# mhamilton723/STEGO

Hardware: NVIDIA H100
Metric: train-step images/sec (higher is better)
Workload: dtype bf16

## Files before the change

include/stego_b200.h:

```cpp
#ifndef STEGO_B200_H_
#define STEGO_B200_H_

#ifdef __cplusplus
extern "C" {
#endif

#define STEGO_API

STEGO_API int stego_version(void);
STEGO_API const char* stego_last_error(void);
STEGO_API long long stego_launch_count(void);

STEGO_API int stego_gemm_bf16(const void* A, int lda, int a_mn_major, const void* B, int ldb, int b_mn_major,
                              int M, int N, int K, void* out, int ldo, int out_bf16, const float* bias, int act,
                              const float* residual, int ldr, int row_div, int splits, int atomic_out,
                              void* stream);

STEGO_API int stego_gemm_bf16_batched(const void* A, int lda, long long a_batch_stride, int a_mn_major, const void* B,
                                      int ldb, long long b_batch_stride, int b_mn_major, int batch, int M, int N, int K,
                                      void* out, int ldo, long long out_batch_stride, int out_bf16, const float* bias,
                                      int act, void* stream);

STEGO_API int stego_vit_patchify(const float* img, void* out_bf16, int B, int H, int W, int patch, void* stream);
STEGO_API int stego_vit_patchify_bf16(const void* img_bf16, void* out_bf16, int B, int H, int W, int patch,
                                      void* stream);
STEGO_API int stego_vit_patchify_tta(const void* img, int img_is_bf16, void* out_bf16, int B, int H, int W, int patch,
                                     void* stream);
STEGO_API int stego_vit_cls_rows(float* x, const float* cls_token, const float* pos_embed, int B, int ntok, int E,
                                 void* stream);
STEGO_API int stego_layernorm_bf16(const float* x, const float* gamma, const float* beta, void* out_bf16, int rows,
                                   int E, float eps, int drop_cls_ntok, void* stream);
STEGO_API int stego_layernorm_gap(const float* x, const float* gamma, const float* beta, float* out, int B, int ntok,
                                  int E, float eps, void* stream);
STEGO_API int stego_linear_rows_f32(const float* x, const void* w_bf16, int ldw, const float* bias, float* out, int B,
                                    int N, int K, void* stream);
STEGO_API int stego_attention_fwd(const void* qkv, void* out, int B, int N, int E, int heads, void* stream);
STEGO_API int stego_attention_probs(const void* qkv, float* probs, int B, int N, int E, int heads, void* stream);

STEGO_API int stego_sample_norm_fwd(const void* src, const void* src_pos, int src_is_bf16, long long stride_b,
                                    long long stride_c, long long stride_y, long long stride_x,
                                    const float* chan_scale, const float* chan_scale_pos, const float* coords1,
                                    const float* coords2, const long long* perms, void* tiles, int B, int C,
                                    int Cpad, int H, int W, int feature_samples, int nslots, int perms_are_raw_randperm,
                                    void* stream);
STEGO_API int stego_sample_labels_fwd(const void* label, const void* label_pos, int label_bytes, const float* coords1,
                                      const float* coords2, const long long* perms, void* tiles, int B, int n_classes,
                                      int Cpad, int H, int W, int feature_samples, int nslots,
                                      int perms_are_raw_randperm, void* stream);
STEGO_API int stego_corr_loss_fwd(const void* feat_tiles, const void* code_tiles, int B, int feature_samples, int E,
                                  int D, int nslots, int ncalls, const int* slot_of_call_host,
                                  const float* shifts_host, int pointwise, int zero_clamp, int stabilize,
                                  float* partials, float* stats, float* cd_out, float* fdc_out, float* loss_out,
                                  void* stream);
STEGO_API int stego_corr_loss_bwd(const void* feat_tiles, const void* code_tiles, int B, int feature_samples, int E,
                                  int D, int nslots, int ncalls, const int* slot_of_call_host,
                                  const float* shifts_host, int pointwise, int zero_clamp, int stabilize,
                                  const float* stats, const float* gscale, const float* gelem, const float* gcd,
                                  float* dtiles, void* stream);
STEGO_API int stego_sample_norm_bwd(const float* code, const float* code_pos, long long stride_b, long long stride_c,
                                    long long stride_y, long long stride_x, const float* coords1,
                                    const float* coords2, const long long* perms, const float* dtiles, float* dcode,
                                    float* dcode_pos, int B, int C, int H, int W, int feature_samples, int nslots,
                                    int perms_are_raw_randperm, void* stream);

STEGO_API int stego_corr_loss_tiled_fwd(const void* feat_tiles, const void* code_tiles, int B, int feature_samples,
                                        int E, int D, int nslots, int ncalls, const int* slot_of_call_host,
                                        const float* shifts_host, int pointwise, int zero_clamp, int stabilize,
                                        float* row_partials, float* row_means, float* stats, float* cd_out,
                                        float* fdc_out, float* loss_out, void* stream);
STEGO_API int stego_corr_loss_tiled_bwd(const void* feat_tiles, const void* code_tiles, int B, int feature_samples,
                                        int E, int D, int nslots, int ncalls, const int* slot_of_call_host,
                                        const float* shifts_host, int pointwise, int zero_clamp, int stabilize,
                                        const float* stats, const float* row_means, const float* gscale,
                                        const float* gelem, const float* gcd, float* dtiles, void* stream);

STEGO_API int stego_salience_counts(const void* salience, const void* salience_pos, int mask_bytes, int B, int H, int W,
                                    int* counts, void* stream);
STEGO_API int stego_salience_coords(const void* salience, const void* salience_pos, int mask_bytes, int B, int H, int W,
                                    int feature_samples, long long seed, const long long* offsets,
                                    const void* draws_u32, const float* u_reg1, const float* u_reg2,
                                    const float* u_keep, float* coords1, float* coords2, void* scratch, void* stream);
STEGO_API long long stego_salience_scratch_bytes(int B, int H, int W);

STEGO_API int stego_aug_record_words(void);
STEGO_API long long stego_aug_scratch_bytes(int B, int size);
STEGO_API int stego_aug_views(const float* img, long long stride_b, long long stride_c, long long stride_y,
                              long long stride_x, int B, int H, int W, int size, const int* records, void* scratch,
                              float* img_aug, float* coord_aug, void* stream);

STEGO_API int stego_frames_rgb8(const void* staging_host, const void* staging_dev, long long bytes,
                                long long table_words, int B, int res, float mean0, float mean1, float mean2,
                                float std0, float std1, float std2, float* out, void* stream);
STEGO_API int stego_labels_u8(const void* staging_host, const void* staging_dev, long long bytes,
                              long long table_words, int B, int res, const long long* lut, long long* out, void* stream);
STEGO_API int stego_frames_store_rgb8(const void* staging_host, const void* staging_dev, long long bytes,
                                      long long table_words, int B, int res, unsigned char* store, long long n,
                                      long long r0, void* stream);
STEGO_API int stego_labels_store_u8(const void* staging_host, const void* staging_dev, long long bytes,
                                    long long table_words, int B, int res, unsigned char* store, long long n,
                                    long long r0, void* stream);
STEGO_API int stego_dataset_batch(const unsigned char* images, const unsigned char* labels, long long n, int res,
                                  const long long* index, int count, const long long* lut, float mean0, float mean1,
                                  float mean2, float std0, float std1, float std2, int out_bf16, int mask_kind,
                                  void* img, long long* label, void* mask, void* stream);
STEGO_API int stego_evalset_batch(const unsigned char* images, const unsigned char* labels, long long n, int res,
                                  const long long* index, int count, const long long* lut, float mean0, float mean1,
                                  float mean2, float std0, float std1, float std2, int out_bf16, int mask_kind,
                                  void* img, long long* label, void* mask, void* stream);
STEGO_API int stego_store_rows_u8(const void* staging_host, const void* staging_dev, long long bytes,
                                  long long table_words, int B, int channels, unsigned char* store,
                                  long long store_bytes, void* stream);
STEGO_API int stego_store_batch_window(const unsigned char* images, long long image_bytes,
                                       const unsigned char* labels, long long label_bytes, const long long* rows,
                                       long long n, int res, const long long* record, int count,
                                       const long long* lut, float mean0, float mean1, float mean2, float std0,
                                       float std1, float std2, int out_bf16, int mask_kind, void* img,
                                       long long* label, void* mask, void* stream);

STEGO_API int stego_jpeg_crops_codec(const void* staging_host, const void* staging_dev, long long bytes,
                                     long long table_words, int count, unsigned char* workspace,
                                     long long workspace_bytes, void* stream);
STEGO_API int stego_jpeg_crops_store_rgb8(const void* staging_host, const void* staging_dev, long long bytes,
                                          long long table_words, int count, int res, const unsigned char* workspace,
                                          long long workspace_bytes, unsigned char* store, long long n, long long r0,
                                          void* stream);

STEGO_API int stego_tb_tables(double* edges, float* thresholds);
STEGO_API int stego_tb_histogram(const float* values, long long n, const float* thresholds, long long* counts,
                                 double* cta_partials, double* stats, void* stream);
STEGO_API int stego_corr_loss_fwd_hist(const void* feat_tiles, const void* code_tiles, int B, int feature_samples,
                                       int E, int D, int nslots, int ncalls, const int* slot_of_call_host,
                                       const float* shifts_host, int pointwise, int zero_clamp, int stabilize,
                                       float* partials, float* stats, float* cd_out, float* fdc_out, float* loss_out,
                                       const float* thresholds, long long* hist_counts, double* hist_cta_partials,
                                       double* hist_stats, void* stream);
STEGO_API int stego_corr_loss_tiled_fwd_hist(const void* feat_tiles, const void* code_tiles, int B,
                                             int feature_samples, int E, int D, int nslots, int ncalls,
                                             const int* slot_of_call_host, const float* shifts_host, int pointwise,
                                             int zero_clamp, int stabilize, float* row_partials, float* row_means,
                                             float* stats, float* cd_out, float* fdc_out, float* loss_out,
                                             const float* thresholds, long long* hist_counts,
                                             double* hist_cta_partials, double* hist_stats, void* stream);

#define STEGO_PR_BINS 4096
STEGO_API int stego_sample_label_ids(const void* label, int label_bytes, const float* coords1, const float* coords2,
                                     int* ids, int B, int n_classes, int H, int W, int feature_samples, void* stream);
STEGO_API int stego_corr_pr(const void* feat_tiles, const void* code_tiles, const int* ids, long long* counts, int B,
                            int feature_samples, int E, int D, void* stream);

STEGO_API int stego_heatmap_prep_target(const void* target, int target_is_bf16, long long stride_b, long long stride_c,
                                        long long stride_y, long long stride_x, int B, int E, int h, int w, int Epad,
                                        void* ops, float* inv_norm, void* stream);
STEGO_API int stego_heatmap_sample_queries(const void* feats, int feats_is_bf16, long long stride_b, long long stride_c,
                                           long long stride_y, long long stride_x, const float* points, int B, int P,
                                           int E, int h, int w, int Epad, int nseg, void* ops, void* stream);
STEGO_API int stego_heatmap_finish(float* corr, const float* inv_norm, int B, int P, int hw, void* stream);
STEGO_API int stego_heatmap_upsample(const float* in, float* out, long long n, int h, int w, int H, int W, void* stream);

STEGO_API int stego_head_dropout3(const void* feat_bf16, const float* mask1, const float* mask2, const float* mask3,
                                  void* out1, void* out2, void* out3, int B, int hw, int E, void* stream);
STEGO_API int stego_cast_pad_bf16(const float* in, int ld_in, int C, void* out_bf16, int ld_out, long long rows,
                                  void* stream);
STEGO_API int stego_relu_bwd_bf16(const float* dh, const void* h_bf16, void* out_bf16, long long n, void* stream);
STEGO_API int stego_colsum(const void* in, int in_is_bf16, int ld, int C, long long rows, float* out, void* stream);
STEGO_API int stego_adam_step(float* param, const float* grad, float* exp_avg, float* exp_avg_sq, long long n,
                              double lr, double beta1, double beta2, double eps, int step, float grad_scale,
                              void* stream);

STEGO_API int stego_step_losses(const float* corr_stats, int ncalls, const float* call_weights_host,
                                const float* extra0, const float* extra1, float* out4, void* stream);

STEGO_API int stego_cluster_lookup_fwd(const float* x, long long stride_b, long long stride_c, long long stride_pix,
                                       const float* clusters, int B, int C, int n_classes, long long npix,
                                       int use_alpha, float alpha, long long* assign, float* probs, float* log_probs,
                                       float* loss_out, float* scratch, void* stream);
STEGO_API int stego_cluster_lookup_bwd(const float* x, long long stride_b, long long stride_c, long long stride_pix,
                                       const float* clusters, int B, int C, int n_classes, long long npix,
                                       int use_alpha, float alpha, const float* grad_loss_dev,
                                       float* dnc_scratch, float* dclusters, void* stream);
STEGO_API int stego_linear_probe_ce(const float* code, long long ld_code, int C, const float* W, const float* bias,
                                    int n_classes, const void* label, int label_bytes, int B, int h, int w, int H,
                                    int Wimg, float* logits_scratch, float* dlogits_scratch, float* partials_scratch,
                                    float* loss_out, float grad_loss, float* dW, float* db, void* stream);
STEGO_API int stego_linear_probe_ce_wide(const float* code, long long ld_code, int C, const float* W, const float* bias,
                                         int n_classes, const void* label, int label_bytes, int B, int h, int w, int H,
                                         int Wimg, float* logits_scratch, float* dlogits_scratch,
                                         long long* dfix_scratch, float* partials_scratch, float* loss_out,
                                         float grad_loss, float* dW, float* db, void* stream);
STEGO_API int stego_cluster_lookup_wide(const float* x, long long ld_x, long long rows, int C, const float* clusters,
                                        int n_classes, int* assign_scratch, float* inv_scratch, float* partials_scratch,
                                        float* loss_out, float* dnc_scratch, float* dclusters, void* stream);

STEGO_API int stego_eval_probes(const float* code, const float* code_flip, long long ld_code, int C, int B, int h, int w,
                                int H, int W, const float* lin_weight, const float* lin_bias, int n_lin,
                                const float* clusters, int n_clu, float alpha, float* lr_scratch, float* lin_log_probs,
                                float* clu_log_probs, unsigned char* lin_argmax, unsigned char* clu_argmax,
                                const void* label, int label_bytes, int n_label_classes, long long* lin_confusion,
                                long long* clu_confusion, void* stream);
STEGO_API int stego_eval_probes_mosaic(const float* code, const float* code_flip, long long ld_code, int C, int B, int h,
                                       int w, int H, int W, const float* lin_weight, const float* lin_bias, int n_lin,
                                       const float* clusters, int n_clu, float alpha, float* lr_scratch,
                                       float* lin_log_probs, float* clu_log_probs, unsigned char* lin_argmax,
                                       unsigned char* clu_argmax, const void* label, int label_bytes,
                                       int n_label_classes, long long* lin_confusion, long long* clu_confusion,
                                       int tile0, int tile_rows, int tiles_per_row, long long pitch, void* stream);

STEGO_API int stego_knn_topk(const float* feats, int n, int E, int k, void* planes_scratch, long long* idx_out,
                             float* val_out, void* stream);
STEGO_API int stego_knn_prep(const float* feats, int n, int E, void* planes, void* stream);
STEGO_API int stego_knn_topk_rows(const void* planes, int n, int E, int k, int row0, int nrows, long long* idx_out,
                                  float* val_out, void* stream);

STEGO_API int stego_crf_lattice(int H, int W, int d, float sxy, float srgb, const unsigned char* image, long long* keys,
                                float* bary, void* stream);
STEGO_API int stego_crf_unary(const float* logits, float* unary, float* Q, long long N, int C, void* stream);
STEGO_API int stego_crf_norm(int d, long long N, int M, const int* offset, const float* bary, const int* rowptr,
                             const int* slots, const int* n1, const int* n2, float* values, float* values_tmp,
                             float* norm_out, void* stream);
STEGO_API int stego_crf_mean_field(int B, long long N, int n_lin, int n_clu, int n_iter, const float* unary, float* Q,
                                   const int* off_g, const float* bary_g, const int* rowptr_g, const int* slots_g,
                                   const int* n1_g, const int* n2_g, const float* norm_g, int Mg,
                                   const int* off_b, const float* bary_b, const int* rowptr_b, const int* slots_b,
                                   const int* n1_b, const int* n2_b, const float* norm_b, int Mb, float w_g,
                                   float w_b, float* val_g, float* tmp_g, float* val_b, float* tmp_b, float* lin_q,
                                   float* clu_q, unsigned char* lin_pred, unsigned char* clu_pred,
                                   const void* label, int label_bytes, int n_label_classes, long long* lin_conf,
                                   long long* clu_conf, void* stream);

STEGO_API int stego_eval_crf_unary(const float* code, const float* code_flip, long long ld_code, int C, int B, int h, int w,
                                   int H, int W, const float* lin_weight, const float* lin_bias, int n_lin,
                                   const float* clusters, int n_clu, float alpha, float* lr_scratch, float* unary, float* Q,
                                   void* stream);
STEGO_API int stego_eval_crf_unary_mosaic(const float* code, const float* code_flip, long long ld_code, int C, int B,
                                          int h, int w, int H, int W, const float* lin_weight, const float* lin_bias,
                                          int n_lin, const float* clusters, int n_clu, float alpha, float* lr_scratch,
                                          float* unary, float* Q, int probes, int tile0, int tile_rows,
                                          int tiles_per_row, long long pitch, void* stream);

STEGO_API int stego_eval_probes_bf16(const void* code, const void* code_flip, long long ld_code, int C, int B, int h,
                                     int w, int H, int W, const float* lin_weight, const float* lin_bias, int n_lin,
                                     const float* clusters, int n_clu, float alpha, float* lr_scratch,
                                     float* lin_log_probs, float* clu_log_probs, unsigned char* lin_argmax,
                                     unsigned char* clu_argmax, const void* label, int label_bytes,
                                     int n_label_classes, long long* lin_confusion, long long* clu_confusion,
                                     void* stream);
STEGO_API int stego_eval_probes_mosaic_bf16(const void* code, const void* code_flip, long long ld_code, int C, int B,
                                            int h, int w, int H, int W, const float* lin_weight, const float* lin_bias,
                                            int n_lin, const float* clusters, int n_clu, float alpha,
                                            float* lr_scratch, float* lin_log_probs, float* clu_log_probs,
                                            unsigned char* lin_argmax, unsigned char* clu_argmax, const void* label,
                                            int label_bytes, int n_label_classes, long long* lin_confusion,
                                            long long* clu_confusion, int tile0, int tile_rows, int tiles_per_row,
                                            long long pitch, void* stream);
STEGO_API int stego_eval_crf_unary_bf16(const void* code, const void* code_flip, long long ld_code, int C, int B, int h,
                                        int w, int H, int W, const float* lin_weight, const float* lin_bias, int n_lin,
                                        const float* clusters, int n_clu, float alpha, float* lr_scratch, float* unary,
                                        float* Q, void* stream);
STEGO_API int stego_eval_crf_unary_mosaic_bf16(const void* code, const void* code_flip, long long ld_code, int C, int B,
                                               int h, int w, int H, int W, const float* lin_weight,
                                               const float* lin_bias, int n_lin, const float* clusters, int n_clu,
                                               float alpha, float* lr_scratch, float* unary, float* Q, int probes,
                                               int tile0, int tile_rows, int tiles_per_row, long long pitch,
                                               void* stream);

STEGO_API int stego_crf_loss_fwd(const float* guidance, long long g_sb, long long g_sc, long long g_sy, long long g_sx, int Cg,
                                 const float* clusters, long long c_sb, long long c_sc, long long c_sy, long long c_sx, int C,
                                 const long long* coords, int B, int n, int H, int W, float alpha, float beta, float gamma,
                                 float w1, float w2, float shift, float* sel, float* gsel, int* pos, float* out, void* stream);
STEGO_API int stego_crf_loss_bwd(const float* grad_out, const float* sel, const float* gsel, const int* pos,
                                 const long long* coords, int B, int C, int n, float alpha, float beta, float gamma, float w1,
                                 float w2, float shift, float* dsel, float* dclusters, long long c_sb, long long c_sc,
                                 long long c_sy, long long c_sx, void* stream);

STEGO_API int stego_cosine_fwd(const float* a, long long a_sb, long long a_sc, long long a_sy, long long a_sx, const float* b,
                               long long b_sb, long long b_sc, long long b_sy, long long b_sx, int B, int C, int H, int W,
                               float eps, float* cosv, float* norma, float* normb, void* stream);
STEGO_API int stego_cosine_bwd(const float* a, long long a_sb, long long a_sc, long long a_sy, long long a_sx, const float* b,
                               long long b_sb, long long b_sc, long long b_sy, long long b_sx, int B, int C, int H, int W,
                               float eps, const float* cosv, const float* norma, const float* normb, const float* grad_cos,
                               float* da, float* db, void* stream);

STEGO_API int stego_aug_align_fwd(const float* coord_aug, int S, const float* code, long long sb, long long sc,
                                  long long sy, long long sx, int B, int C, int h, float* grid, float* sampled,
                                  void* stream);
STEGO_API int stego_aug_align_bwd(const float* grid, const float* dsampled, int B, int C, int h, float* dcode,
                                  long long sb, long long sc, long long sy, long long sx, void* stream);
STEGO_API int stego_aug_align_loss(const float* cosv, long long n, float weight, float* loss, float* total, void* stream);

STEGO_API int stego_rec_fwd(const float* code, long long ldc, const void* feat, long long ldf, const float* m3, int hw,
                            const float* weight, const float* bias, long long M, int E, int D, float* cosv, float* nr,
                            float* nf, void* stream);
STEGO_API long long stego_rec_scratch_bytes(long long M, int E, int D);
STEGO_API int stego_rec_bwd(const float* code, long long ldc, const void* feat, long long ldf, const float* m3, int hw,
                            const float* weight, const float* bias, long long M, int E, int D, const float* cosv,
                            const float* nr, const float* nf, const float* dcos, float* dcode, long long ldd,
                            float* scratch, long long scratch_bytes, float* dweight, float* dbias, void* stream);

STEGO_API int stego_crf_guidance(const float* img, long long sb, long long sc, long long sy, long long sx, int Cg, int H,
                                 int W, const long long* coords, int B, int n, int S, float* gsel, int* pos, void* stream);
STEGO_API int stego_crf_mean_fwd(const float* code, long long sb, long long sc, long long sy, long long sx, int C, int h,
                                 int w, const long long* coords, int B, int n, int S, float alpha, float beta, float gamma,
                                 float w1, float w2, float shift, const float* gsel, const int* pos, float* raw,
                                 float* sel, float* nrm, double* tile_sum, void* stream);
STEGO_API int stego_crf_mean_loss(const double* tile_sum, int B, int n, float weight, float* loss, float* total,
                                  void* stream);
STEGO_API int stego_crf_mean_bwd(const float* gscalar, const float* sel, const float* nrm, const float* gsel,
                                 const int* pos, const long long* coords, int B, int C, int n, int h, int w, int S,
                                 float alpha, float beta, float gamma, float w1, float w2, float shift, float* dsel,
                                 float* dcode, long long sb, long long sc, long long sy, long long sx, void* stream);

STEGO_API int stego_p2p_alloc(long long bytes, long long* ptr_out, unsigned char* handle_out);
STEGO_API int stego_p2p_open(const unsigned char* handle, long long* ptr_out);
STEGO_API int stego_p2p_close(long long ptr);
STEGO_API int stego_p2p_free(long long ptr);
STEGO_API int stego_p2p_publish(const float* grad, long long n, float* export_slot, const long long* peer_flags, int rank,
                                int world, int epoch, int* status, int timeout_ms, void* stream);
STEGO_API int stego_p2p_adam(const long long* peer_exports, int world, float* param, float* grad, float* exp_avg,
                             float* exp_avg_sq, long long n, const double* group_desc, int ngroups, float grad_scale,
                             void* stream);

#ifdef __cplusplus
}
#endif
#endif
```

stego_b200/_lib.py:

```python
from __future__ import annotations

import ctypes
import gc
import os
import re
import threading
from typing import Dict, List, Tuple

import torch

_HERE = os.path.dirname(os.path.abspath(__file__))
LIB_PATH = os.path.join(_HERE, "libstego_b200.so")
HEADER_PATH = os.path.join(_HERE, "..", "include", "stego_b200.h")

_lib = None
replayed_launches = 0

_CTYPES = {
    "int": ctypes.c_int,
    "float": ctypes.c_float,
    "double": ctypes.c_double,
    "long long": ctypes.c_longlong,
    "void*": ctypes.c_void_p,
    "const void*": ctypes.c_void_p,
    "const float*": ctypes.c_void_p,
    "float*": ctypes.c_void_p,
    "const long long*": ctypes.c_void_p,
    "long long*": ctypes.c_void_p,
    "const int*": ctypes.c_void_p,
    "int*": ctypes.c_void_p,
    "const char*": ctypes.c_char_p,
    "unsigned char*": ctypes.c_void_p,
    "const unsigned char*": ctypes.c_void_p,
    "const double*": ctypes.c_void_p,
    "double*": ctypes.c_void_p,
}


def header_prototypes() -> Dict[str, Tuple[str, List[str]]]:
    text = open(HEADER_PATH).read()
    text = re.sub(r"/\*.*?\*/", "", text, flags=re.S)
    text = re.sub(r"//[^\n]*", "", text)
    text = re.sub(r"^\s*#[^\n]*", "", text, flags=re.M)
    protos: Dict[str, Tuple[str, List[str]]] = {}
    for m in re.finditer(r"STEGO_API\s+([\w\s\*]+?)\s*\b(stego_\w+)\s*\(([^;]*?)\)\s*;", text, flags=re.S):
        ret, name, args = m.group(1).strip(), m.group(2), m.group(3).strip()
        arg_types: List[str] = []
        if args and args != "void":
            for a in args.split(","):
                a = " ".join(a.split())
                t = re.sub(r"\s*\b\w+$", "", a).strip()
                t = t.replace(" *", "*")
                arg_types.append(t)
        protos[name] = (ret.replace(" *", "*"), arg_types)
    return protos


def load():
    global _lib
    if _lib is not None:
        return _lib
    if not os.path.exists(LIB_PATH):
        raise RuntimeError(
            f"stego_b200: {LIB_PATH} is missing. Build it with `python -m stego_b200.build` "
            "(or __graft_entry__.build()). There is no CPU / eager fallback for the hot path.")
    lib = ctypes.CDLL(LIB_PATH)
    for name, (ret, args) in header_prototypes().items():
        fn = getattr(lib, name)
        fn.restype = _CTYPES[ret]
        fn.argtypes = [_CTYPES[a] for a in args]
    _lib = lib
    return lib


def launch_count() -> int:
    return int(load().stego_launch_count()) + replayed_launches


_CAPTURE_LOCK = threading.Lock()


_CAPTURE_STREAMS: Dict[int, torch.cuda.Stream] = {}


def capture_stream(device: torch.device) -> torch.cuda.Stream:
    if device.index not in _CAPTURE_STREAMS:
        _CAPTURE_STREAMS[device.index] = torch.cuda.Stream(device=device)
    return _CAPTURE_STREAMS[device.index]


class Graph:

    def __init__(self, fn):
        self.device = torch.device("cuda", torch.cuda.current_device())
        with _CAPTURE_LOCK, torch.cuda.device(self.device):
            self._capture(fn)

    def _capture(self, fn):
        torch.cuda.synchronize()
        gc.collect()
        enabled = gc.isenabled()
        gc.disable()
        try:
            self.graph = torch.cuda.CUDAGraph()
            n0 = load().stego_launch_count()
            with torch.cuda.graph(self.graph, stream=capture_stream(self.device)):
                self.result = fn()
            self.launches = load().stego_launch_count() - n0
        finally:
            if enabled:
                gc.enable()

    def replay(self) -> None:
        global replayed_launches
        if torch.cuda.current_device() == self.device.index:
            self.graph.replay()
        else:
            with torch.cuda.device(self.device):
                self.graph.replay()
        replayed_launches += self.launches


def last_error() -> str:
    return load().stego_last_error().decode("utf-8", "replace")


def check(rc: int, what: str) -> None:
    if rc != 0:
        raise RuntimeError(f"stego_b200.{what} failed with status {rc}: {last_error()}")


def ptr(t) -> int:
    if t is None:
        return 0
    return t.data_ptr()


def stream() -> int:
    return torch.cuda.current_stream().cuda_stream


def require_cuda(*tensors) -> None:
    for t in tensors:
        if t is not None and not t.is_cuda:
            raise RuntimeError("stego_b200: hot-path tensors must live on a CUDA device (no CPU fallback)")
```

stego_b200/csrc/attention.cu:

```cuda
#include <stdlib.h>

#include "common.cuh"
#include "host_util.h"

namespace stego {

constexpr int ATT_BQ = 128;
constexpr int ATT_BKV = 64;
constexpr int ATT_D = 64;
constexpr int ATT_STAGES = 4;
constexpr int ATT_THREADS = 288;

constexpr uint32_t ATT_Q_BYTES = 128 * 64 * 2;
constexpr uint32_t ATT_KV_BYTES = 64 * 64 * 2;
constexpr uint32_t ATT_SMEM_Q = 0;
constexpr uint32_t ATT_SMEM_KV = ATT_Q_BYTES;
constexpr uint32_t ATT_SMEM_BAR = ATT_SMEM_KV + ATT_STAGES * 2 * ATT_KV_BYTES;
constexpr uint32_t ATT_SMEM_TOTAL = ATT_SMEM_BAR + 128;

struct AttnParams {
  int N;
  int E;
  float scale_log2e;
};

__global__ void __launch_bounds__(ATT_THREADS, 2)
attention_fwd_kernel(const __grid_constant__ CUtensorMap tmQKV, const __grid_constant__ CUtensorMap tmOut, AttnParams p) {
  extern __shared__ __align__(1024) uint8_t smem[];
  if ((smem_u32(smem) & 1023u) != 0u) __trap();
  uint64_t* bars = reinterpret_cast<uint64_t*>(smem + ATT_SMEM_BAR);
  uint64_t* q_full = bars;
  uint64_t* kv_full = bars + 1;
  uint64_t* kv_empty = kv_full + ATT_STAGES;

  const int warp = threadIdx.x >> 5;
  const int lane = threadIdx.x & 31;
  const int q0 = blockIdx.x * ATT_BQ;
  const int head = blockIdx.y;
  const int img = blockIdx.z;
  const int nkv = (p.N + ATT_BKV - 1) / ATT_BKV;

  if (threadIdx.x == 0) {
    mbar_init(q_full, 1);
    for (int s = 0; s < ATT_STAGES; ++s) {
      mbar_init(&kv_full[s], 1);
      mbar_init(&kv_empty[s], 2);
    }
    fence_barrier_init();
  }
  __syncthreads();

  if (warp == 8) {
    if (lane == 0) {
      tma_prefetch_desc(&tmQKV);
      tma_prefetch_desc(&tmOut);
      mbar_arrive_expect_tx(q_full, ATT_Q_BYTES);
      tma_load_3d(smem + ATT_SMEM_Q, &tmQKV, q_full, head * ATT_D, q0, img);
      tma_load_3d(smem + ATT_SMEM_Q + ATT_Q_BYTES / 2, &tmQKV, q_full, head * ATT_D, q0 + 64, img);
      uint32_t stage = 0, phase = 0;
      for (int j = 0; j < nkv; ++j) {
        mbar_wait(&kv_empty[stage], phase ^ 1u);
        uint8_t* sk = smem + ATT_SMEM_KV + stage * 2 * ATT_KV_BYTES;
        mbar_arrive_expect_tx(&kv_full[stage], 2 * ATT_KV_BYTES);
        tma_load_3d(sk, &tmQKV, &kv_full[stage], p.E + head * ATT_D, j * ATT_BKV, img);
        tma_load_3d(sk + ATT_KV_BYTES, &tmQKV, &kv_full[stage], 2 * p.E + head * ATT_D, j * ATT_BKV, img);
        if (++stage == ATT_STAGES) { stage = 0; phase ^= 1u; }
      }
    }
    return;
  }

  const int wg = warp >> 2;
  const int wq = warp & 3;
  const bool leader = (threadIdx.x & 127) == 0;
  const float c = p.scale_log2e;
  constexpr uint32_t DESC_HI = smem_desc_hi_sw128(1024);
  uint8_t* sq = smem + ATT_SMEM_Q + wg * (ATT_Q_BYTES / 2);
  const uint32_t q_lo = smem_desc_lo(smem_u32(sq), 16);
  const uint32_t k_lo0 = smem_desc_lo(smem_u32(smem + ATT_SMEM_KV), 16);
  const uint32_t v_lo0 = smem_desc_lo(smem_u32(smem + ATT_SMEM_KV + ATT_KV_BYTES), 8192);
  float o[32];
#pragma unroll
  for (int i = 0; i < 32; ++i) o[i] = 0.f;
  float m_run[2] = {-INFINITY, -INFINITY}, l_run[2] = {0.f, 0.f};
  mbar_wait(q_full, 0);
  uint32_t stage = 0, phase = 0;
  for (int j = 0; j < nkv; ++j) {
    mbar_wait(&kv_full[stage], phase);
    const uint32_t k_lo = k_lo0 + stage * ((2 * ATT_KV_BYTES) >> 4);
    const uint32_t v_lo = v_lo0 + stage * ((2 * ATT_KV_BYTES) >> 4);
    float s[32];
    wgmma_fence();
#pragma unroll
    for (uint32_t k = 0; k < ATT_D / 16; ++k)
      wgmma_ss<64, 0, 0>(s, smem_desc_join(q_lo + k * 2, DESC_HI), smem_desc_join(k_lo + k * 2, DESC_HI), k > 0 ? 1u : 0u);
    wgmma_commit();
    wgmma_wait<0>();
    fence_operands(s);
    const int valid = p.N - j * ATT_BKV;
    if (valid < ATT_BKV) {
#pragma unroll
      for (int i = 0; i < 32; ++i)
        if (8 * (i >> 2) + 2 * (lane & 3) + (i & 1) >= valid) s[i] = -INFINITY;
    }
    float alpha[2], mc[2];
#pragma unroll
    for (int h = 0; h < 2; ++h) {
      float mx = -INFINITY;
#pragma unroll
      for (int i = 0; i < 8; ++i) mx = fmaxf(mx, fmaxf(s[4 * i + 2 * h], s[4 * i + 2 * h + 1]));
      mx = fmaxf(mx, __shfl_xor_sync(0xffffffffu, mx, 1));
      mx = fmaxf(mx, __shfl_xor_sync(0xffffffffu, mx, 2));
      const float m_new = fmaxf(m_run[h], mx);
      alpha[h] = ex2_approx((m_run[h] - m_new) * c);
      m_run[h] = m_new;
      mc[h] = m_new * c;
    }
    uint32_t a[4][4];
    float rs[2] = {0.f, 0.f};
#pragma unroll
    for (int i = 0; i < 8; ++i) {
#pragma unroll
      for (int h = 0; h < 2; ++h) {
        const float e0 = ex2_approx(fmaf(s[4 * i + 2 * h], c, -mc[h]));
        const float e1 = ex2_approx(fmaf(s[4 * i + 2 * h + 1], c, -mc[h]));
        rs[h] += e0 + e1;
        a[i >> 1][(i & 1) * 2 + h] = pack_bf16x2(e0, e1);
      }
    }
#pragma unroll
    for (int h = 0; h < 2; ++h) l_run[h] = l_run[h] * alpha[h] + rs[h];
#pragma unroll
    for (int i = 0; i < 32; ++i) o[i] *= alpha[(i >> 1) & 1];
    wgmma_fence();
#pragma unroll
    for (uint32_t kk = 0; kk < ATT_BKV / 16; ++kk)
      wgmma_rs_n64<1>(o, a[kk], smem_desc_join(v_lo + kk * (2048u >> 4), DESC_HI), 1u);
    wgmma_commit();
    wgmma_wait<0>();
    fence_operands(o);
    if (leader) mbar_arrive(&kv_empty[stage]);
    if (++stage == ATT_STAGES) { stage = 0; phase ^= 1u; }
  }
  float inv[2];
#pragma unroll
  for (int h = 0; h < 2; ++h) {
    float l = l_run[h];
    l += __shfl_xor_sync(0xffffffffu, l, 1);
    l += __shfl_xor_sync(0xffffffffu, l, 2);
    inv[h] = __fdividef(1.0f, l);
  }
#pragma unroll
  for (int i = 0; i < 8; ++i) {
#pragma unroll
    for (int h = 0; h < 2; ++h) {
      const uint32_t r = static_cast<uint32_t>(wq * 16 + (lane >> 2) + 8 * h);
      const uint32_t off = sw128_offset(r, static_cast<uint32_t>(i)) + 4u * static_cast<uint32_t>(lane & 3);
      *reinterpret_cast<uint32_t*>(sq + off) = pack_bf16x2(o[4 * i + 2 * h] * inv[h], o[4 * i + 2 * h + 1] * inv[h]);
    }
  }
  fence_proxy_async_smem();
  asm volatile("bar.sync %0, 128;\n" ::"r"(wg + 1) : "memory");
  if (leader) {
    tma_store_3d(sq, &tmOut, head * ATT_D, q0 + wg * 64, img);
    tma_commit_group();
    tma_wait_group_read<0>();
  }
}

constexpr int PRB_STAGES = 4;
constexpr int PRB_PITCH = 72;
constexpr uint32_t PRB_SMEM_K = ATT_Q_BYTES;
constexpr uint32_t PRB_SMEM_STAGE = PRB_SMEM_K + PRB_STAGES * ATT_KV_BYTES;
constexpr uint32_t PRB_WARP_STAGE_BYTES = 16 * PRB_PITCH * 4;
constexpr uint32_t PRB_SMEM_BAR = PRB_SMEM_STAGE + 8 * PRB_WARP_STAGE_BYTES;
constexpr uint32_t PRB_SMEM_TOTAL = PRB_SMEM_BAR + 128;

__device__ __forceinline__ void st_global_cs(float* p, float v) {
  asm volatile("st.global.cs.f32 [%0], %1;\n" ::"l"(p), "f"(v) : "memory");
}

__global__ void __launch_bounds__(ATT_THREADS, 2)
attention_probs_kernel(const __grid_constant__ CUtensorMap tmQKV, float* __restrict__ probs, AttnParams p) {
  extern __shared__ __align__(1024) uint8_t smem[];
  if ((smem_u32(smem) & 1023u) != 0u) __trap();
  uint64_t* bars = reinterpret_cast<uint64_t*>(smem + PRB_SMEM_BAR);
  uint64_t* q_full = bars;
  uint64_t* k_full = bars + 1;
  uint64_t* k_empty = k_full + PRB_STAGES;

  const int warp = threadIdx.x >> 5;
  const int lane = threadIdx.x & 31;
  const int q0 = blockIdx.x * ATT_BQ;
  const int head = blockIdx.y;
  const int img = blockIdx.z;
  const int nkv = (p.N + ATT_BKV - 1) / ATT_BKV;

  if (threadIdx.x == 0) {
    mbar_init(q_full, 1);
    for (int s = 0; s < PRB_STAGES; ++s) {
      mbar_init(&k_full[s], 1);
      mbar_init(&k_empty[s], 2);
    }
    fence_barrier_init();
  }
  __syncthreads();

  if (warp == 8) {
    if (lane == 0) {
      tma_prefetch_desc(&tmQKV);
      mbar_arrive_expect_tx(q_full, ATT_Q_BYTES);
      tma_load_3d(smem, &tmQKV, q_full, head * ATT_D, q0, img);
      tma_load_3d(smem + ATT_Q_BYTES / 2, &tmQKV, q_full, head * ATT_D, q0 + 64, img);
      uint32_t stage = 0, phase = 0;
      for (int j = 0; j < 2 * nkv; ++j) {
        mbar_wait(&k_empty[stage], phase ^ 1u);
        mbar_arrive_expect_tx(&k_full[stage], ATT_KV_BYTES);
        tma_load_3d(smem + PRB_SMEM_K + stage * ATT_KV_BYTES, &tmQKV, &k_full[stage], p.E + head * ATT_D,
                    (j < nkv ? j : j - nkv) * ATT_BKV, img);
        if (++stage == PRB_STAGES) { stage = 0; phase ^= 1u; }
      }
    }
    return;
  }

  const int wg = warp >> 2;
  const int wq = warp & 3;
  const bool leader = (threadIdx.x & 127) == 0;
  const float c = p.scale_log2e;
  constexpr uint32_t DESC_HI = smem_desc_hi_sw128(1024);
  const uint32_t q_lo = smem_desc_lo(smem_u32(smem + wg * (ATT_Q_BYTES / 2)), 16);
  const uint32_t k_lo0 = smem_desc_lo(smem_u32(smem + PRB_SMEM_K), 16);
  float* stage_tile = reinterpret_cast<float*>(smem + PRB_SMEM_STAGE + warp * PRB_WARP_STAGE_BYTES);
  const int row0 = q0 + wg * 64 + wq * 16;
  float m_run[2] = {-INFINITY, -INFINITY}, l_run[2] = {0.f, 0.f};
  float inv[2] = {0.f, 0.f};
  mbar_wait(q_full, 0);
  uint32_t stage = 0, phase = 0;
  for (int j = 0; j < 2 * nkv; ++j) {
    const bool store_pass = j >= nkv;
    const int kt = store_pass ? j - nkv : j;
    mbar_wait(&k_full[stage], phase);
    const uint32_t k_lo = k_lo0 + stage * (ATT_KV_BYTES >> 4);
    float s[32];
    wgmma_fence();
#pragma unroll
    for (uint32_t k = 0; k < ATT_D / 16; ++k)
      wgmma_ss<64, 0, 0>(s, smem_desc_join(q_lo + k * 2, DESC_HI), smem_desc_join(k_lo + k * 2, DESC_HI), k > 0 ? 1u : 0u);
    wgmma_commit();
    wgmma_wait<0>();
    fence_operands(s);
    if (leader) mbar_arrive(&k_empty[stage]);
    if (++stage == PRB_STAGES) { stage = 0; phase ^= 1u; }
    const int valid = p.N - kt * ATT_BKV;
    if (!store_pass) {
      if (valid < ATT_BKV) {
#pragma unroll
        for (int i = 0; i < 32; ++i)
          if (8 * (i >> 2) + 2 * (lane & 3) + (i & 1) >= valid) s[i] = -INFINITY;
      }
#pragma unroll
      for (int h = 0; h < 2; ++h) {
        float mx = -INFINITY;
#pragma unroll
        for (int i = 0; i < 8; ++i) mx = fmaxf(mx, fmaxf(s[4 * i + 2 * h], s[4 * i + 2 * h + 1]));
        mx = fmaxf(mx, __shfl_xor_sync(0xffffffffu, mx, 1));
        mx = fmaxf(mx, __shfl_xor_sync(0xffffffffu, mx, 2));
        const float m_new = fmaxf(m_run[h], mx);
        const float alpha = ex2_approx((m_run[h] - m_new) * c);
        float rs = 0.f;
#pragma unroll
        for (int i = 0; i < 8; ++i)
          rs += ex2_approx((s[4 * i + 2 * h] - m_new) * c) + ex2_approx((s[4 * i + 2 * h + 1] - m_new) * c);
        l_run[h] = l_run[h] * alpha + rs;
        m_run[h] = m_new;
      }
      if (kt == nkv - 1) {
#pragma unroll
        for (int h = 0; h < 2; ++h) {
          float l = l_run[h];
          l += __shfl_xor_sync(0xffffffffu, l, 1);
          l += __shfl_xor_sync(0xffffffffu, l, 2);
          inv[h] = __frcp_rn(l);
        }
      }
      continue;
    }
    __syncwarp();
#pragma unroll
    for (int i = 0; i < 8; ++i) {
#pragma unroll
      for (int h = 0; h < 2; ++h) {
        const float p0 = ex2_approx((s[4 * i + 2 * h] - m_run[h]) * c) * inv[h];
        const float p1 = ex2_approx((s[4 * i + 2 * h + 1] - m_run[h]) * c) * inv[h];
        float2* dst = reinterpret_cast<float2*>(stage_tile + ((lane >> 2) + 8 * h) * PRB_PITCH + 8 * i + 2 * (lane & 3));
        *dst = make_float2(p0, p1);
      }
    }
    __syncwarp();
    const int nrows = min(16, p.N - row0);
    const size_t plane = (static_cast<size_t>(img) * gridDim.y + head) * static_cast<size_t>(p.N);
    float* out = probs + (plane + static_cast<size_t>(row0)) * static_cast<size_t>(p.N) + static_cast<size_t>(kt) * ATT_BKV;
#pragma unroll 4
    for (int r = 0; r < nrows; ++r) {
      float* orow = out + static_cast<size_t>(r) * static_cast<size_t>(p.N);
      if (lane < valid) st_global_cs(orow + lane, stage_tile[r * PRB_PITCH + lane]);
      if (lane + 32 < valid) st_global_cs(orow + lane + 32, stage_tile[r * PRB_PITCH + lane + 32]);
    }
  }
}

}

using namespace stego;

extern "C" int stego_attention_fwd(const void* qkv, void* out, int B, int N, int E, int heads, void* stream_) {
  cudaStream_t stream = reinterpret_cast<cudaStream_t>(stream_);
  STEGO_CHECK_ARG(qkv && out, "stego_attention_fwd: null pointer");
  STEGO_CHECK_ARG(B > 0 && N > 0 && heads > 0, "stego_attention_fwd: bad sizes");
  STEGO_CHECK_ARG(E == heads * ATT_D, "stego_attention_fwd: head_dim must be 64 (E=%d heads=%d)", E, heads);
  STEGO_CHECK_ARG((reinterpret_cast<uintptr_t>(out) & 15u) == 0, "stego_attention_fwd: out not 16-byte aligned");
  CUtensorMap tm;
  uint64_t dims[3] = {(uint64_t)3 * E, (uint64_t)N, (uint64_t)B};
  uint64_t str[2] = {(uint64_t)3 * E * 2, (uint64_t)N * 3 * E * 2};
  uint32_t box[3] = {64, 64, 1};
  int rc = make_tmap_bf16(&tm, qkv, 3, dims, str, box);
  if (rc != STEGO_OK) return rc;
  CUtensorMap tmo;
  uint64_t odims[3] = {(uint64_t)E, (uint64_t)N, (uint64_t)B};
  uint64_t ostr[2] = {(uint64_t)E * 2, (uint64_t)N * E * 2};
  if ((rc = make_tmap_bf16(&tmo, out, 3, odims, ostr, box)) != STEGO_OK) return rc;
  if ((rc = opt_in_smem<attention_fwd_kernel>(ATT_SMEM_TOTAL, "attention_fwd_kernel")) != STEGO_OK) return rc;
  AttnParams p;
  p.N = N;
  p.E = E;
  p.scale_log2e = 0.125f * 1.4426950408889634f;
  dim3 grid((N + ATT_BQ - 1) / ATT_BQ, heads, B);
  attention_fwd_kernel<<<grid, ATT_THREADS, ATT_SMEM_TOTAL, stream>>>(tm, tmo, p);
  STEGO_CHECK_LAUNCH("attention_fwd_kernel");
  return STEGO_OK;
}

extern "C" int stego_attention_probs(const void* qkv, float* probs, int B, int N, int E, int heads, void* stream_) {
  cudaStream_t stream = reinterpret_cast<cudaStream_t>(stream_);
  STEGO_CHECK_ARG(qkv && probs, "stego_attention_probs: null pointer");
  STEGO_CHECK_ARG(B > 0 && N > 0 && heads > 0, "stego_attention_probs: bad sizes");
  STEGO_CHECK_ARG(B <= 65535 && heads <= 65535, "stego_attention_probs: B and heads must be <= 65535");
  STEGO_CHECK_ARG(E == heads * ATT_D, "stego_attention_probs: head_dim must be 64 (E=%d heads=%d)", E, heads);
  STEGO_CHECK_ARG((reinterpret_cast<uintptr_t>(probs) & 3u) == 0, "stego_attention_probs: probs not 4-byte aligned");
  CUtensorMap tm;
  uint64_t dims[3] = {(uint64_t)3 * E, (uint64_t)N, (uint64_t)B};
  uint64_t str[2] = {(uint64_t)3 * E * 2, (uint64_t)N * 3 * E * 2};
  uint32_t box[3] = {64, 64, 1};
  int rc = make_tmap_bf16(&tm, qkv, 3, dims, str, box);
  if (rc != STEGO_OK) return rc;
  if ((rc = opt_in_smem<attention_probs_kernel>(PRB_SMEM_TOTAL, "attention_probs_kernel")) != STEGO_OK) return rc;
  AttnParams p;
  p.N = N;
  p.E = E;
  p.scale_log2e = 0.125f * 1.4426950408889634f;
  dim3 grid((N + ATT_BQ - 1) / ATT_BQ, heads, B);
  attention_probs_kernel<<<grid, ATT_THREADS, PRB_SMEM_TOTAL, stream>>>(tm, probs, p);
  STEGO_CHECK_LAUNCH("attention_probs_kernel");
  return STEGO_OK;
}
```

stego_b200/csrc/common.cuh:

```cuda
#pragma once
#include <cuda.h>
#include <cuda_bf16.h>
#include <cuda_runtime.h>
#include <stdint.h>
#include <stdio.h>

namespace stego {

typedef __nv_bfloat16 bf16;

__device__ __forceinline__ uint32_t smem_u32(const void* p) {
  return static_cast<uint32_t>(__cvta_generic_to_shared(p));
}
__device__ __forceinline__ uint32_t lane_id() { return threadIdx.x & 31u; }

__device__ __forceinline__ float warp_sum(float v) {
#pragma unroll
  for (int o = 16; o > 0; o >>= 1) v += __shfl_xor_sync(0xffffffffu, v, o);
  return v;
}
__device__ __forceinline__ float warp_max(float v) {
#pragma unroll
  for (int o = 16; o > 0; o >>= 1) v = fmaxf(v, __shfl_xor_sync(0xffffffffu, v, o));
  return v;
}

__device__ __forceinline__ void mbar_init(uint64_t* bar, uint32_t count) {
  asm volatile("mbarrier.init.shared::cta.b64 [%0], %1;\n" ::"r"(smem_u32(bar)), "r"(count) : "memory");
}
__device__ __forceinline__ void fence_barrier_init() {
  asm volatile("fence.mbarrier_init.release.cluster;\n" ::: "memory");
}
__device__ __forceinline__ void fence_proxy_async_smem() {
  asm volatile("fence.proxy.async.shared::cta;\n" ::: "memory");
}
__device__ __forceinline__ void mbar_arrive(uint64_t* bar) {
  asm volatile("mbarrier.arrive.shared::cta.b64 _, [%0];\n" ::"r"(smem_u32(bar)) : "memory");
}
__device__ __forceinline__ void mbar_arrive_expect_tx(uint64_t* bar, uint32_t bytes) {
  asm volatile("mbarrier.arrive.expect_tx.shared::cta.b64 _, [%0], %1;\n" ::"r"(smem_u32(bar)), "r"(bytes)
               : "memory");
}
__device__ __forceinline__ bool mbar_try_wait(uint64_t* bar, uint32_t parity) {
  uint32_t ok;
  asm volatile(
      "{\n\t.reg .pred P1;\n\t"
      "mbarrier.try_wait.parity.shared::cta.b64 P1, [%1], %2, %3;\n\t"
      "selp.b32 %0, 1, 0, P1;\n\t}\n"
      : "=r"(ok)
      : "r"(smem_u32(bar)), "r"(parity), "r"(1000000u)
      : "memory");
  return ok != 0;
}

__device__ __forceinline__ bool mbar_test_wait(uint64_t* bar, uint32_t parity) {
  uint32_t ok;
  asm volatile(
      "{\n\t.reg .pred P1;\n\t"
      "mbarrier.test_wait.parity.shared::cta.b64 P1, [%1], %2;\n\t"
      "selp.b32 %0, 1, 0, P1;\n\t}\n"
      : "=r"(ok)
      : "r"(smem_u32(bar)), "r"(parity)
      : "memory");
  return ok != 0;
}

#ifndef STEGO_MBAR_TIMEOUT_NS
#define STEGO_MBAR_TIMEOUT_NS 4000000000ull
#endif
__device__ __forceinline__ uint64_t globaltimer_ns() {
  uint64_t t;
  asm volatile("mov.u64 %0, %%globaltimer;\n" : "=l"(t));
  return t;
}
__device__ __forceinline__ void mbar_wait(uint64_t* bar, uint32_t parity) {
  if (mbar_test_wait(bar, parity)) return;
  if (mbar_try_wait(bar, parity)) return;
  uint32_t spins = 0;
  uint64_t t0 = 0;
  while (!mbar_try_wait(bar, parity)) {
    if ((++spins & 0x3Fu) == 0) {
      const uint64_t now = globaltimer_ns();
      if (t0 == 0) {
        t0 = now;
      } else if (now - t0 > STEGO_MBAR_TIMEOUT_NS) {
        __trap();
      }
    }
  }
}

__device__ __forceinline__ void tma_prefetch_desc(const CUtensorMap* m) {
  asm volatile("prefetch.tensormap [%0];\n" ::"l"(reinterpret_cast<uint64_t>(m)) : "memory");
}
__device__ __forceinline__ void tma_load_2d(void* smem_dst, const CUtensorMap* m, uint64_t* bar, int c0, int c1) {
  asm volatile(
      "cp.async.bulk.tensor.2d.shared::cluster.global.mbarrier::complete_tx::bytes [%0], [%1, {%3, %4}], [%2];\n" ::"r"(
          smem_u32(smem_dst)),
      "l"(reinterpret_cast<uint64_t>(m)), "r"(smem_u32(bar)), "r"(c0), "r"(c1)
      : "memory");
}
__device__ __forceinline__ void tma_load_3d(void* smem_dst, const CUtensorMap* m, uint64_t* bar, int c0, int c1,
                                            int c2) {
  asm volatile(
      "cp.async.bulk.tensor.3d.shared::cluster.global.mbarrier::complete_tx::bytes [%0], [%1, {%3, %4, %5}], "
      "[%2];\n" ::"r"(smem_u32(smem_dst)),
      "l"(reinterpret_cast<uint64_t>(m)), "r"(smem_u32(bar)), "r"(c0), "r"(c1), "r"(c2)
      : "memory");
}

__device__ __forceinline__ void tma_prefetch_l2_2d(const CUtensorMap* m, int c0, int c1) {
  asm volatile("cp.async.bulk.prefetch.tensor.2d.L2.global [%0, {%1, %2}];\n" ::"l"(reinterpret_cast<uint64_t>(m)),
               "r"(c0), "r"(c1)
               : "memory");
}

__device__ __forceinline__ void tma_store_3d(uint32_t smem_src, const CUtensorMap* m, int c0, int c1, int c2) {
  asm volatile("cp.async.bulk.tensor.3d.global.shared::cta.bulk_group [%0, {%2, %3, %4}], [%1];\n" ::"l"(
                   reinterpret_cast<uint64_t>(m)),
               "r"(smem_src), "r"(c0), "r"(c1), "r"(c2)
               : "memory");
}
__device__ __forceinline__ void tma_store_3d(const void* smem_src, const CUtensorMap* m, int c0, int c1, int c2) {
  tma_store_3d(smem_u32(smem_src), m, c0, c1, c2);
}
__device__ __forceinline__ void tma_reduce_add_3d(uint32_t smem_src, const CUtensorMap* m, int c0, int c1, int c2) {
  asm volatile("cp.reduce.async.bulk.tensor.3d.global.shared::cta.add.bulk_group [%0, {%2, %3, %4}], [%1];\n" ::"l"(
                   reinterpret_cast<uint64_t>(m)),
               "r"(smem_src), "r"(c0), "r"(c1), "r"(c2)
               : "memory");
}

__device__ __forceinline__ void st_shared_b32(uint32_t addr, uint32_t v) {
  asm volatile("st.shared.b32 [%0], %1;\n" ::"r"(addr), "r"(v) : "memory");
}
__device__ __forceinline__ void st_shared_v2_f32(uint32_t addr, float a, float b) {
  asm volatile("st.shared.v2.f32 [%0], {%1, %2};\n" ::"r"(addr), "f"(a), "f"(b) : "memory");
}
__device__ __forceinline__ void tma_commit_group() { asm volatile("cp.async.bulk.commit_group;\n" ::: "memory"); }
template <int kPending>
__device__ __forceinline__ void tma_wait_group_read() {
  asm volatile("cp.async.bulk.wait_group.read %0;\n" ::"n"(kPending) : "memory");
}
template <int kPending>
__device__ __forceinline__ void tma_wait_group() {
  asm volatile("cp.async.bulk.wait_group %0;\n" ::"n"(kPending) : "memory");
}

__device__ __forceinline__ void named_bar_sync(int id, int threads) {
  asm volatile("bar.sync %0, %1;\n" ::"r"(id), "r"(threads) : "memory");
}

__device__ __forceinline__ void wgmma_fence() { asm volatile("wgmma.fence.sync.aligned;\n" ::: "memory"); }
__device__ __forceinline__ void wgmma_commit() { asm volatile("wgmma.commit_group.sync.aligned;\n" ::: "memory"); }
template <int kPending>
__device__ __forceinline__ void wgmma_wait() {
  asm volatile("wgmma.wait_group.sync.aligned %0;\n" ::"n"(kPending) : "memory");
}
template <int kN>
__device__ __forceinline__ void fence_operands(float (&d)[kN]) {
#pragma unroll
  for (int i = 0; i < kN; ++i) asm volatile("" : "+f"(d[i])::"memory");
}

template <int kTransA, int kTransB>
__device__ __forceinline__ void wgmma_ss_n64(float (&d)[32], uint64_t desc_a, uint64_t desc_b, uint32_t accumulate) {
  asm volatile(
      "{\n\t.reg .pred p;\n\tsetp.ne.b32 p, %34, 0;\n\t"
      "wgmma.mma_async.sync.aligned.m64n64k16.f32.bf16.bf16 {%0, %1, %2, %3, %4, %5, %6, %7, %8, %9, %10, %11, %12, %13, %14, %15, %16, %17, %18, %19, %20, %21, %22, %23, %24, %25, %26, %27, %28, %29, %30, %31}, %32, %33, p, 1, 1, %35, %36;\n\t}\n"
      : "+f"(d[0]), "+f"(d[1]), "+f"(d[2]), "+f"(d[3]), "+f"(d[4]), "+f"(d[5]), "+f"(d[6]), "+f"(d[7]), "+f"(d[8]), "+f"(d[9]), "+f"(d[10]), "+f"(d[11]), "+f"(d[12]), "+f"(d[13]), "+f"(d[14]), "+f"(d[15]), "+f"(d[16]), "+f"(d[17]), "+f"(d[18]), "+f"(d[19]), "+f"(d[20]), "+f"(d[21]), "+f"(d[22]), "+f"(d[23]), "+f"(d[24]), "+f"(d[25]), "+f"(d[26]), "+f"(d[27]), "+f"(d[28]), "+f"(d[29]), "+f"(d[30]), "+f"(d[31])
      : "l"(desc_a), "l"(desc_b), "r"(accumulate), "n"(kTransA), "n"(kTransB));
}

template <int kTransA, int kTransB>
__device__ __forceinline__ void wgmma_ss_n128(float (&d)[64], uint64_t desc_a, uint64_t desc_b, uint32_t accumulate) {
  asm volatile(
      "{\n\t.reg .pred p;\n\tsetp.ne.b32 p, %66, 0;\n\t"
      "wgmma.mma_async.sync.aligned.m64n128k16.f32.bf16.bf16 {%0, %1, %2, %3, %4, %5, %6, %7, %8, %9, %10, %11, %12, %13, %14, %15, %16, %17, %18, %19, %20, %21, %22, %23, %24, %25, %26, %27, %28, %29, %30, %31, %32, %33, %34, %35, %36, %37, %38, %39, %40, %41, %42, %43, %44, %45, %46, %47, %48, %49, %50, %51, %52, %53, %54, %55, %56, %57, %58, %59, %60, %61, %62, %63}, %64, %65, p, 1, 1, %67, %68;\n\t}\n"
      : "+f"(d[0]), "+f"(d[1]), "+f"(d[2]), "+f"(d[3]), "+f"(d[4]), "+f"(d[5]), "+f"(d[6]), "+f"(d[7]), "+f"(d[8]), "+f"(d[9]), "+f"(d[10]), "+f"(d[11]), "+f"(d[12]), "+f"(d[13]), "+f"(d[14]), "+f"(d[15]), "+f"(d[16]), "+f"(d[17]), "+f"(d[18]), "+f"(d[19]), "+f"(d[20]), "+f"(d[21]), "+f"(d[22]), "+f"(d[23]), "+f"(d[24]), "+f"(d[25]), "+f"(d[26]), "+f"(d[27]), "+f"(d[28]), "+f"(d[29]), "+f"(d[30]), "+f"(d[31]), "+f"(d[32]), "+f"(d[33]), "+f"(d[34]), "+f"(d[35]), "+f"(d[36]), "+f"(d[37]), "+f"(d[38]), "+f"(d[39]), "+f"(d[40]), "+f"(d[41]), "+f"(d[42]), "+f"(d[43]), "+f"(d[44]), "+f"(d[45]), "+f"(d[46]), "+f"(d[47]), "+f"(d[48]), "+f"(d[49]), "+f"(d[50]), "+f"(d[51]), "+f"(d[52]), "+f"(d[53]), "+f"(d[54]), "+f"(d[55]), "+f"(d[56]), "+f"(d[57]), "+f"(d[58]), "+f"(d[59]), "+f"(d[60]), "+f"(d[61]), "+f"(d[62]), "+f"(d[63])
      : "l"(desc_a), "l"(desc_b), "r"(accumulate), "n"(kTransA), "n"(kTransB));
}

template <int kTransA, int kTransB>
__device__ __forceinline__ void wgmma_ss_n256(float (&d)[128], uint64_t desc_a, uint64_t desc_b, uint32_t accumulate) {
  asm volatile(
      "{\n\t.reg .pred p;\n\tsetp.ne.b32 p, %130, 0;\n\t"
      "wgmma.mma_async.sync.aligned.m64n256k16.f32.bf16.bf16 {%0, %1, %2, %3, %4, %5, %6, %7, %8, %9, %10, %11, %12, %13, %14, %15, %16, %17, %18, %19, %20, %21, %22, %23, %24, %25, %26, %27, %28, %29, %30, %31, %32, %33, %34, %35, %36, %37, %38, %39, %40, %41, %42, %43, %44, %45, %46, %47, %48, %49, %50, %51, %52, %53, %54, %55, %56, %57, %58, %59, %60, %61, %62, %63, %64, %65, %66, %67, %68, %69, %70, %71, %72, %73, %74, %75, %76, %77, %78, %79, %80, %81, %82, %83, %84, %85, %86, %87, %88, %89, %90, %91, %92, %93, %94, %95, %96, %97, %98, %99, %100, %101, %102, %103, %104, %105, %106, %107, %108, %109, %110, %111, %112, %113, %114, %115, %116, %117, %118, %119, %120, %121, %122, %123, %124, %125, %126, %127}, %128, %129, p, 1, 1, %131, %132;\n\t}\n"
      : "+f"(d[0]), "+f"(d[1]), "+f"(d[2]), "+f"(d[3]), "+f"(d[4]), "+f"(d[5]), "+f"(d[6]), "+f"(d[7]), "+f"(d[8]), "+f"(d[9]), "+f"(d[10]), "+f"(d[11]), "+f"(d[12]), "+f"(d[13]), "+f"(d[14]), "+f"(d[15]), "+f"(d[16]), "+f"(d[17]), "+f"(d[18]), "+f"(d[19]), "+f"(d[20]), "+f"(d[21]), "+f"(d[22]), "+f"(d[23]), "+f"(d[24]), "+f"(d[25]), "+f"(d[26]), "+f"(d[27]), "+f"(d[28]), "+f"(d[29]), "+f"(d[30]), "+f"(d[31]), "+f"(d[32]), "+f"(d[33]), "+f"(d[34]), "+f"(d[35]), "+f"(d[36]), "+f"(d[37]), "+f"(d[38]), "+f"(d[39]), "+f"(d[40]), "+f"(d[41]), "+f"(d[42]), "+f"(d[43]), "+f"(d[44]), "+f"(d[45]), "+f"(d[46]), "+f"(d[47]), "+f"(d[48]), "+f"(d[49]), "+f"(d[50]), "+f"(d[51]), "+f"(d[52]), "+f"(d[53]), "+f"(d[54]), "+f"(d[55]), "+f"(d[56]), "+f"(d[57]), "+f"(d[58]), "+f"(d[59]), "+f"(d[60]), "+f"(d[61]), "+f"(d[62]), "+f"(d[63]), "+f"(d[64]), "+f"(d[65]), "+f"(d[66]), "+f"(d[67]), "+f"(d[68]), "+f"(d[69]), "+f"(d[70]), "+f"(d[71]), "+f"(d[72]), "+f"(d[73]), "+f"(d[74]), "+f"(d[75]), "+f"(d[76]), "+f"(d[77]), "+f"(d[78]), "+f"(d[79]), "+f"(d[80]), "+f"(d[81]), "+f"(d[82]), "+f"(d[83]), "+f"(d[84]), "+f"(d[85]), "+f"(d[86]), "+f"(d[87]), "+f"(d[88]), "+f"(d[89]), "+f"(d[90]), "+f"(d[91]), "+f"(d[92]), "+f"(d[93]), "+f"(d[94]), "+f"(d[95]), "+f"(d[96]), "+f"(d[97]), "+f"(d[98]), "+f"(d[99]), "+f"(d[100]), "+f"(d[101]), "+f"(d[102]), "+f"(d[103]), "+f"(d[104]), "+f"(d[105]), "+f"(d[106]), "+f"(d[107]), "+f"(d[108]), "+f"(d[109]), "+f"(d[110]), "+f"(d[111]), "+f"(d[112]), "+f"(d[113]), "+f"(d[114]), "+f"(d[115]), "+f"(d[116]), "+f"(d[117]), "+f"(d[118]), "+f"(d[119]), "+f"(d[120]), "+f"(d[121]), "+f"(d[122]), "+f"(d[123]), "+f"(d[124]), "+f"(d[125]), "+f"(d[126]), "+f"(d[127])
      : "l"(desc_a), "l"(desc_b), "r"(accumulate), "n"(kTransA), "n"(kTransB));
}

template <int kTransB>
__device__ __forceinline__ void wgmma_rs_n64(float (&d)[32], const uint32_t (&a)[4], uint64_t desc_b, uint32_t accumulate) {
  asm volatile(
      "{\n\t.reg .pred p;\n\tsetp.ne.b32 p, %37, 0;\n\t"
      "wgmma.mma_async.sync.aligned.m64n64k16.f32.bf16.bf16 {%0, %1, %2, %3, %4, %5, %6, %7, %8, %9, %10, %11, %12, %13, %14, %15, %16, %17, %18, %19, %20, %21, %22, %23, %24, %25, %26, %27, %28, %29, %30, %31}, {%32, %33, %34, %35}, %36, p, 1, 1, %38;\n\t}\n"
      : "+f"(d[0]), "+f"(d[1]), "+f"(d[2]), "+f"(d[3]), "+f"(d[4]), "+f"(d[5]), "+f"(d[6]), "+f"(d[7]), "+f"(d[8]), "+f"(d[9]), "+f"(d[10]), "+f"(d[11]), "+f"(d[12]), "+f"(d[13]), "+f"(d[14]), "+f"(d[15]), "+f"(d[16]), "+f"(d[17]), "+f"(d[18]), "+f"(d[19]), "+f"(d[20]), "+f"(d[21]), "+f"(d[22]), "+f"(d[23]), "+f"(d[24]), "+f"(d[25]), "+f"(d[26]), "+f"(d[27]), "+f"(d[28]), "+f"(d[29]), "+f"(d[30]), "+f"(d[31])
      : "r"(a[0]), "r"(a[1]), "r"(a[2]), "r"(a[3]), "l"(desc_b), "r"(accumulate), "n"(kTransB));
}

template <int N, int kTransA, int kTransB>
__device__ __forceinline__ void wgmma_ss(float (&d)[N / 2], uint64_t desc_a, uint64_t desc_b, uint32_t accumulate) {
  static_assert(N == 64 || N == 128 || N == 256, "wgmma_ss: N must be 64, 128 or 256");
  if constexpr (N == 64) wgmma_ss_n64<kTransA, kTransB>(d, desc_a, desc_b, accumulate);
  else if constexpr (N == 128) wgmma_ss_n128<kTransA, kTransB>(d, desc_a, desc_b, accumulate);
  else wgmma_ss_n256<kTransA, kTransB>(d, desc_a, desc_b, accumulate);
}

template <uint32_t kRegs>
__device__ __forceinline__ void warpgroup_reg_alloc() { asm volatile("setmaxnreg.inc.sync.aligned.u32 %0;\n" ::"n"(kRegs)); }
template <uint32_t kRegs>
__device__ __forceinline__ void warpgroup_reg_dealloc() { asm volatile("setmaxnreg.dec.sync.aligned.u32 %0;\n" ::"n"(kRegs)); }

__device__ __forceinline__ float ex2_approx(float x) {
  float y;
  asm("ex2.approx.ftz.f32 %0, %1;\n" : "=f"(y) : "f"(x));
  return y;
}

__device__ __forceinline__ float ex2_approx_v(float x) {
  float y;
  asm volatile("ex2.approx.ftz.f32 %0, %1;\n" : "=f"(y) : "f"(x));
  return y;
}

__device__ __forceinline__ uint32_t smem_desc_lo(uint32_t smem_addr, uint32_t lbo_bytes) {
  return ((smem_addr & 0x3FFFFu) >> 4) | (((lbo_bytes >> 4) & 0x3FFFu) << 16);
}
__host__ __device__ constexpr uint32_t smem_desc_hi_sw128(uint32_t sbo_bytes) {
  return ((sbo_bytes >> 4) & 0x3FFFu) | (1u << 30);
}
__device__ __forceinline__ uint64_t smem_desc_join(uint32_t lo, uint32_t hi) {
  return (static_cast<uint64_t>(hi) << 32) | lo;
}

__device__ __forceinline__ uint32_t sw128_offset(uint32_t row, uint32_t chunk16) {
  return row * 128u + ((chunk16 ^ (row & 7u)) << 4);
}

__device__ __forceinline__ uint64_t pack_f32x2(float lo, float hi) {
  uint64_t r;
  asm("mov.b64 %0, {%1, %2};\n" : "=l"(r) : "f"(lo), "f"(hi));
  return r;
}
__device__ __forceinline__ void unpack_f32x2(uint64_t v, float& lo, float& hi) {
  asm("mov.b64 {%0, %1}, %2;\n" : "=f"(lo), "=f"(hi) : "l"(v));
}
__device__ __forceinline__ uint64_t fma_f32x2(uint64_t a, uint64_t b, uint64_t c) {
  float a0, a1, b0, b1, c0, c1;
  unpack_f32x2(a, a0, a1); unpack_f32x2(b, b0, b1); unpack_f32x2(c, c0, c1);
  return pack_f32x2(__fmaf_rn(a0, b0, c0), __fmaf_rn(a1, b1, c1));
}
__device__ __forceinline__ uint64_t add_f32x2(uint64_t a, uint64_t b) {
  float a0, a1, b0, b1;
  unpack_f32x2(a, a0, a1); unpack_f32x2(b, b0, b1);
  return pack_f32x2(__fadd_rn(a0, b0), __fadd_rn(a1, b1));
}
__device__ __forceinline__ uint64_t mul_f32x2(uint64_t a, uint64_t b) {
  float a0, a1, b0, b1;
  unpack_f32x2(a, a0, a1); unpack_f32x2(b, b0, b1);
  return pack_f32x2(__fmul_rn(a0, b0), __fmul_rn(a1, b1));
}

__device__ __forceinline__ uint32_t pack_bf16x2(float lo, float hi) {
  __nv_bfloat162 v = __floats2bfloat162_rn(lo, hi);
  return *reinterpret_cast<uint32_t*>(&v);
}

struct AdamCoef {
  float b1, c1, b2, c2;
  float step_size;
  float sqrt_bc2;
  float eps;
};
inline AdamCoef adam_coef(double lr, double beta1, double beta2, double eps, double step) {
  AdamCoef c;
  c.b1 = static_cast<float>(beta1);
  c.c1 = static_cast<float>(1.0 - beta1);
  c.b2 = static_cast<float>(beta2);
  c.c2 = static_cast<float>(1.0 - beta2);
  c.step_size = static_cast<float>(lr / (1.0 - pow(beta1, step)));
  c.sqrt_bc2 = static_cast<float>(sqrt(1.0 - pow(beta2, step)));
  c.eps = static_cast<float>(eps);
  return c;
}
__device__ __forceinline__ void adam_elem(float& p, float& m, float& v, float g, const AdamCoef& c) {
  m = __fmaf_rn(c.c1, g, __fmul_rn(m, c.b1));
  v = __fmaf_rn(__fmul_rn(c.c2, g), g, __fmul_rn(v, c.b2));
  const float denom = __fadd_rn(__fdiv_rn(__fsqrt_rn(v), c.sqrt_bc2), c.eps);
  p = __fmaf_rn(-c.step_size, __fdiv_rn(m, denom), p);
}

}
```

stego_b200/csrc/gemm.cu:

```cuda
#include <stdlib.h>
#include <string.h>

#include "common.cuh"
#include "epilogue.cuh"
#include "host_util.h"

namespace stego {

constexpr int GEMM_BM = 128;
constexpr int GEMM_BN = 128;
constexpr int GEMM_BK = 64;
constexpr int GEMM_THREADS = 384;
constexpr uint32_t GEMM_STAGE_BYTES = (GEMM_BM + GEMM_BN) * GEMM_BK * 2;
constexpr uint32_t GEMM_CHUNK_BYTES = GEMM_BM * 128;

struct GemmParams {
  int M, N, K;
  int splits;
  int kb_per_split;
  void* out;
  int ldo;
  int out_bf16;
  const float* bias;
  int act;
  const float* residual;
  int ldr;
  int row_div;
  int atomic;
  int vec_ok;
  int reduce_add;
  int batch;
  long long out_bs;
  long long res_bs;
};

template <int BN>
__device__ __forceinline__ void gemm_bias_act(float (&acc)[BN / 2], const GemmParams& p, int col_base) {
  if (p.bias != nullptr) {
#pragma unroll
    for (int c = 0; c < BN / 8; ++c) {
      const int col = col_base + 8 * c;
      float b0 = 0.f, b1 = 0.f;
      if (col + 1 < p.N && p.vec_ok) {
        const float2 b2 = __ldg(reinterpret_cast<const float2*>(p.bias + col));
        b0 = b2.x; b1 = b2.y;
      } else {
        if (col < p.N) b0 = __ldg(p.bias + col);
        if (col + 1 < p.N) b1 = __ldg(p.bias + col + 1);
      }
      acc[4 * c + 0] += b0; acc[4 * c + 1] += b1;
      acc[4 * c + 2] += b0; acc[4 * c + 3] += b1;
    }
  }
  if (p.act == 1) {
    if (p.out_bf16) {
#pragma unroll
      for (int j = 0; j < BN / 2; j += 8) gelu_erf_poly8(acc + j);
    } else {
#pragma unroll
      for (int j = 0; j < BN / 2; ++j) acc[j] = gelu_erf(acc[j]);
    }
  } else if (p.act == 2) {
#pragma unroll
    for (int j = 0; j < BN / 2; ++j) acc[j] = fmaxf(acc[j], 0.0f);
  }
}

template <int BN>
__device__ __forceinline__ void gemm_store_regs(const float (&acc)[BN / 2], const GemmParams& p, int row_top,
                                                int col_base, int tb) {
  void* const outp = p.out_bf16 ? static_cast<void*>(reinterpret_cast<bf16*>(p.out) + tb * p.out_bs)
                                : static_cast<void*>(reinterpret_cast<float*>(p.out) + tb * p.out_bs);
  const float* const resp = p.residual ? p.residual + tb * p.res_bs : nullptr;
#pragma unroll
  for (int h = 0; h < 2; ++h) {
    const int row = row_top + 8 * h;
    if (row >= p.M) continue;
    int out_row = row, res_row = row;
    if (p.row_div > 0) {
      out_row = row + row / p.row_div + 1;
      res_row = row % p.row_div + 1;
    }
    const size_t obase = static_cast<size_t>(out_row) * p.ldo;
    const size_t rbase = static_cast<size_t>(res_row) * p.ldr;
#pragma unroll
    for (int c = 0; c < BN / 8; ++c) {
      const int col = col_base + 8 * c;
      if (col >= p.N) break;
      const bool two = col + 1 < p.N;
      float x0 = acc[4 * c + 2 * h], x1 = acc[4 * c + 2 * h + 1];
      if (p.atomic) {
        float* o = reinterpret_cast<float*>(outp) + obase + col;
        atomicAdd(o, x0);
        if (two) atomicAdd(o + 1, x1);
        continue;
      }
      const bool vec = two && p.vec_ok;
      if (resp != nullptr) {
        if (vec) {
          const float2 r = *reinterpret_cast<const float2*>(resp + rbase + col);
          x0 += r.x; x1 += r.y;
        } else {
          x0 += resp[rbase + col];
          if (two) x1 += resp[rbase + col + 1];
        }
      }
      if (p.out_bf16) {
        bf16* o = reinterpret_cast<bf16*>(outp) + obase + col;
        if (vec) {
          *reinterpret_cast<uint32_t*>(o) = pack_bf16x2(x0, x1);
        } else {
          o[0] = __float2bfloat16_rn(x0);
          if (two) o[1] = __float2bfloat16_rn(x1);
        }
      } else {
        float* o = reinterpret_cast<float*>(outp) + obase + col;
        if (vec) {
          *reinterpret_cast<float2*>(o) = make_float2(x0, x1);
        } else {
          o[0] = x0;
          if (two) o[1] = x1;
        }
      }
    }
  }
}

template <bool kBf16, int kBufs = 2>
__device__ __forceinline__ void gemm_store_tma(const float (&acc)[2][GEMM_BN / 2], const GemmParams& p,
                                               const CUtensorMap* tm_out, uint32_t stage, int bar_id, bool issuer,
                                               int m0, int n0, int tb) {
  constexpr int kCols = kBf16 ? 64 : 32;
  const int lane = threadIdx.x & 31;
  const int wq = (threadIdx.x >> 5) & 3;
  const uint32_t q = lane & 3;
  const uint32_t swz = (lane >> 2) & 7;
#pragma unroll
  for (int ch = 0; ch < GEMM_BN / kCols; ++ch) {
    const uint32_t buf = stage + (ch % kBufs) * GEMM_CHUNK_BYTES;
    if (issuer) tma_wait_group_read<kBufs - 1>();
    named_bar_sync(bar_id, 128);
    const uint32_t rbase = buf + (16 * wq + (lane >> 2)) * 128u;
#pragma unroll
    for (int h = 0; h < 2; ++h) {
#pragma unroll
      for (int e2 = 0; e2 < 2; ++e2) {
        const uint32_t rp = rbase + (64 * h + 8 * e2) * 128u;
        if constexpr (kBf16) {
#pragma unroll
          for (int j = 0; j < 8; ++j) {
            const int c = 8 * ch + j;
            st_shared_b32(rp + (((uint32_t)j ^ swz) << 4) + 4 * q,
                          pack_bf16x2(acc[h][4 * c + 2 * e2], acc[h][4 * c + 2 * e2 + 1]));
          }
        } else {
#pragma unroll
          for (int j = 0; j < 4; ++j) {
            const int c = 4 * ch + j;
            const uint32_t unit = 2 * j + (q >> 1);
            st_shared_v2_f32(rp + ((unit ^ swz) << 4) + 8 * (q & 1), acc[h][4 * c + 2 * e2],
                             acc[h][4 * c + 2 * e2 + 1]);
          }
        }
      }
    }
    fence_proxy_async_smem();
    named_bar_sync(bar_id, 128);
    if (issuer) {
      const int col = n0 + ch * kCols;
      if (p.reduce_add) tma_reduce_add_3d(buf, tm_out, col, m0, tb);
      else tma_store_3d(buf, tm_out, col, m0, tb);
      tma_commit_group();
    }
  }
}

template <int kStages>
__device__ __forceinline__ void ring_advance(uint32_t& stage, uint32_t& phase, int n) {
  stage += n;
  while (stage >= kStages) { stage -= kStages; phase ^= 1u; }
}

template <int kStages, bool A_MN, bool B_MN, bool kTmaEpi>
__global__ void __launch_bounds__(GEMM_THREADS, 1)
gemm_bf16_kernel(const __grid_constant__ CUtensorMap tmA, const __grid_constant__ CUtensorMap tmB,
                 const __grid_constant__ CUtensorMap tmOut, GemmParams p) {
  constexpr uint32_t A_BYTES = GEMM_BM * GEMM_BK * 2;
  constexpr uint32_t STAGE_BYTES = GEMM_STAGE_BYTES;

  extern __shared__ __align__(1024) uint8_t smem_raw[];
  uint8_t* smem = reinterpret_cast<uint8_t*>((reinterpret_cast<uintptr_t>(smem_raw) + 1023) & ~uintptr_t(1023));
  uint8_t* staging = smem + kStages * STAGE_BYTES;
  uint64_t* full_bar = reinterpret_cast<uint64_t*>(staging + (kTmaEpi ? 4 * GEMM_CHUNK_BYTES : 0));
  uint64_t* empty_bar = full_bar + kStages;
  uint64_t* turn_bar = empty_bar + kStages;

  const int warp = threadIdx.x >> 5;
  const int lane = threadIdx.x & 31;
  const int wg = warp >> 2;

  const int tiles_m = (p.M + GEMM_BM - 1) / GEMM_BM;
  const int tiles_n = (p.N + GEMM_BN - 1) / GEMM_BN;
  const int num_kb = (p.K + GEMM_BK - 1) / GEMM_BK;
  const int tiles_per_batch = tiles_m * tiles_n * p.splits;
  const int total_tiles = tiles_per_batch * p.batch;
  const int sched_start = static_cast<int>(blockIdx.x);
  const int sched_step = static_cast<int>(gridDim.x);

  if (threadIdx.x == 0) {
    tma_prefetch_desc(&tmA);
    tma_prefetch_desc(&tmB);
    if (kTmaEpi) tma_prefetch_desc(&tmOut);
    for (int s = 0; s < kStages; ++s) {
      mbar_init(&full_bar[s], 1);
      mbar_init(&empty_bar[s], 1);
    }
    mbar_init(&turn_bar[0], 1);
    mbar_init(&turn_bar[1], 1);
    fence_barrier_init();
  }
  __syncthreads();

  if (wg == 0) {
    warpgroup_reg_dealloc<40>();
    if (threadIdx.x == 0) {
      uint32_t stage = 0, phase = 0;
      for (int t = sched_start; t < total_tiles; t += sched_step) {
        const int tb = t / tiles_per_batch, tl = t % tiles_per_batch;
        const int split = tl % p.splits;
        const int tn = (tl / p.splits) % tiles_n;
        const int tm = tl / (p.splits * tiles_n);
        const int kb0 = split * p.kb_per_split;
        const int kb1 = min(num_kb, kb0 + p.kb_per_split);
        for (int kb = kb0; kb < kb1; ++kb) {
          mbar_wait(&empty_bar[stage], phase ^ 1u);
          uint8_t* sa = smem + stage * STAGE_BYTES;
          uint8_t* sb = sa + A_BYTES;
          mbar_arrive_expect_tx(&full_bar[stage], STAGE_BYTES);
          if (!A_MN) {
            tma_load_3d(sa, &tmA, &full_bar[stage], kb * GEMM_BK, tm * GEMM_BM, tb);
          } else {
#pragma unroll
            for (int blk = 0; blk < GEMM_BM / 64; ++blk)
              tma_load_3d(sa + blk * 8192, &tmA, &full_bar[stage], tm * GEMM_BM + blk * 64, kb * GEMM_BK, tb);
          }
          if (!B_MN) {
            tma_load_3d(sb, &tmB, &full_bar[stage], kb * GEMM_BK, tn * GEMM_BN, tb);
          } else {
#pragma unroll
            for (int blk = 0; blk < GEMM_BN / 64; ++blk)
              tma_load_3d(sb + blk * 8192, &tmB, &full_bar[stage], tn * GEMM_BN + blk * 64, kb * GEMM_BK, tb);
          }
          if (++stage == kStages) { stage = 0; phase ^= 1u; }
        }
      }
    }
  } else {
    warpgroup_reg_alloc<232>();
    const int mwg = wg - 1;
    constexpr uint32_t DESC_HI = smem_desc_hi_sw128(1024);
    constexpr uint32_t A_KSTEP = A_MN ? (2048u >> 4) : (32u >> 4);
    constexpr uint32_t B_KSTEP = B_MN ? (2048u >> 4) : (32u >> 4);
    constexpr uint32_t A_HALF = 8192u >> 4;
    const uint32_t a_lo0 = smem_desc_lo(smem_u32(smem), 8192u);
    const uint32_t b_lo0 = smem_desc_lo(smem_u32(smem) + A_BYTES, 8192u);
    const bool leader = (threadIdx.x & 127) == 0;
    const int wq = (threadIdx.x >> 5) & 3;
    uint32_t stage = 0, phase = 0;
    float acc[2][GEMM_BN / 2];
    int i = 0;
    for (int t = sched_start; t < total_tiles; t += sched_step, ++i) {
      const int tb = t / tiles_per_batch, tl = t % tiles_per_batch;
      const int split = tl % p.splits;
      const int tn = (tl / p.splits) % tiles_n;
      const int tm = tl / (p.splits * tiles_n);
      const int kb0 = split * p.kb_per_split;
      const int kb1 = min(num_kb, kb0 + p.kb_per_split);
      if ((i & 1) != mwg) {
        ring_advance<kStages>(stage, phase, kb1 - kb0);
        continue;
      }
      if (i > 0) mbar_wait(&turn_bar[mwg], ((i - 1) >> 1) & 1);
#pragma unroll
      for (int j = 0; j < GEMM_BN / 2; ++j) { acc[0][j] = 0.f; acc[1][j] = 0.f; }
      uint32_t prev_stage = 0;
      for (int kb = kb0; kb < kb1; ++kb) {
        mbar_wait(&full_bar[stage], phase);
        const uint32_t a_lo = a_lo0 + stage * (STAGE_BYTES >> 4);
        const uint32_t b_lo = b_lo0 + stage * (STAGE_BYTES >> 4);
        fence_operands(acc[0]);
        fence_operands(acc[1]);
        wgmma_fence();
#pragma unroll
        for (uint32_t k = 0; k < GEMM_BK / 16; ++k) {
          const uint64_t db = smem_desc_join(b_lo + k * B_KSTEP, DESC_HI);
#pragma unroll
          for (uint32_t h = 0; h < 2; ++h)
            wgmma_ss<GEMM_BN, A_MN ? 1 : 0, B_MN ? 1 : 0>(
                acc[h], smem_desc_join(a_lo + h * A_HALF + k * A_KSTEP, DESC_HI), db, 1u);
        }
        wgmma_commit();
        wgmma_wait<1>();
        if (kb > kb0 && leader) mbar_arrive(&empty_bar[prev_stage]);
        prev_stage = stage;
        if (++stage == kStages) { stage = 0; phase ^= 1u; }
      }
      if (leader) mbar_arrive(&turn_bar[mwg ^ 1]);
      wgmma_wait<0>();
      fence_operands(acc[0]);
      fence_operands(acc[1]);
      if (kb1 > kb0 && leader) mbar_arrive(&empty_bar[prev_stage]);
      const int col_base = tn * GEMM_BN + 2 * (lane & 3);
      gemm_bias_act<GEMM_BN>(acc[0], p, col_base);
      gemm_bias_act<GEMM_BN>(acc[1], p, col_base);
      if constexpr (kTmaEpi) {
        const uint32_t st = smem_u32(staging) + mwg * 2 * GEMM_CHUNK_BYTES;
        if (p.out_bf16) gemm_store_tma<true>(acc, p, &tmOut, st, 1 + mwg, leader, tm * GEMM_BM, tn * GEMM_BN, tb);
        else gemm_store_tma<false>(acc, p, &tmOut, st, 1 + mwg, leader, tm * GEMM_BM, tn * GEMM_BN, tb);
      } else {
        const int row_top = tm * GEMM_BM + wq * 16 + (lane >> 2);
        gemm_store_regs<GEMM_BN>(acc[0], p, row_top, col_base, tb);
        gemm_store_regs<GEMM_BN>(acc[1], p, row_top + 64, col_base, tb);
      }
    }
    if (kTmaEpi && leader) tma_wait_group<0>();
  }
}

template <int kStages, bool A_MN, bool B_MN, bool kTmaEpi>
static int launch_gemm(const CUtensorMap& tmA, const CUtensorMap& tmB, const CUtensorMap& tmOut, const GemmParams& p,
                       cudaStream_t stream) {
  constexpr size_t smem = size_t(kStages) * GEMM_STAGE_BYTES + (kTmaEpi ? 4 * GEMM_CHUNK_BYTES : 0) + 1024 + 256;
  static_assert(smem <= 232448, "exceeds the 227 KB of shared memory a CTA can opt into");
  constexpr auto kern = gemm_bf16_kernel<kStages, A_MN, B_MN, kTmaEpi>;
  if (const int rc = opt_in_smem<kern>(smem, "gemm_bf16_kernel"); rc != STEGO_OK) return rc;
  const int tiles_m = (p.M + GEMM_BM - 1) / GEMM_BM;
  const int tiles_n = (p.N + GEMM_BN - 1) / GEMM_BN;
  const int tiles = tiles_m * tiles_n * p.splits * p.batch;
  const int grid = tiles < num_sms() ? tiles : num_sms();
  kern<<<grid, GEMM_THREADS, smem, stream>>>(tmA, tmB, tmOut, p);
  STEGO_CHECK_LAUNCH("gemm_bf16_kernel launch");
  return STEGO_OK;
}

template <bool A_MN, bool B_MN>
static int launch_gemm_epi(bool tma_epi, const CUtensorMap& tmA, const CUtensorMap& tmB, const CUtensorMap& tmOut,
                           const GemmParams& p, cudaStream_t stream) {
  if (tma_epi) return launch_gemm<5, A_MN, B_MN, true>(tmA, tmB, tmOut, p, stream);
  return launch_gemm<6, A_MN, B_MN, false>(tmA, tmB, tmOut, p, stream);
}

constexpr int GEMM_RES_MAX_K = 384;
constexpr uint32_t GEMM_RES_BOX_BYTES = GEMM_BM * GEMM_BK * 2;
constexpr uint32_t GEMM_RES_B_BYTES = (GEMM_RES_MAX_K / GEMM_BK) * GEMM_RES_BOX_BYTES;

template <int kStages, int kBufs>
__global__ void __launch_bounds__(GEMM_THREADS, 1)
gemm_bf16_resident_kernel(const __grid_constant__ CUtensorMap tmA, const __grid_constant__ CUtensorMap tmB,
                          const __grid_constant__ CUtensorMap tmOut, GemmParams p) {
  constexpr uint32_t BOX = GEMM_RES_BOX_BYTES;

  extern __shared__ __align__(1024) uint8_t smem_raw[];
  uint8_t* smem = reinterpret_cast<uint8_t*>((reinterpret_cast<uintptr_t>(smem_raw) + 1023) & ~uintptr_t(1023));
  uint8_t* sb = smem;
  uint8_t* sa = smem + GEMM_RES_B_BYTES;
  uint8_t* staging = sa + kStages * BOX;
  uint64_t* full_bar = reinterpret_cast<uint64_t*>(staging + 2 * kBufs * GEMM_CHUNK_BYTES);
  uint64_t* empty_bar = full_bar + kStages;
  uint64_t* turn_bar = empty_bar + kStages;
  uint64_t* b_bar = turn_bar + 2;

  const int warp = threadIdx.x >> 5;
  const int lane = threadIdx.x & 31;
  const int wg = warp >> 2;

  const int tiles_m = (p.M + GEMM_BM - 1) / GEMM_BM;
  const int tiles_n = (p.N + GEMM_BN - 1) / GEMM_BN;
  const int num_kb = (p.K + GEMM_BK - 1) / GEMM_BK;
  const int tn = static_cast<int>(blockIdx.x) % tiles_n;
  const int tm_start = static_cast<int>(blockIdx.x) / tiles_n;
  const int tm_step = (static_cast<int>(gridDim.x) - tn + tiles_n - 1) / tiles_n;

  if (threadIdx.x == 0) {
    tma_prefetch_desc(&tmA);
    tma_prefetch_desc(&tmB);
    tma_prefetch_desc(&tmOut);
    for (int s = 0; s < kStages; ++s) {
      mbar_init(&full_bar[s], 1);
      mbar_init(&empty_bar[s], 1);
    }
    mbar_init(&turn_bar[0], 1);
    mbar_init(&turn_bar[1], 1);
    mbar_init(b_bar, 1);
    fence_barrier_init();
  }
  __syncthreads();

  if (wg == 0) {
    warpgroup_reg_dealloc<40>();
    if (threadIdx.x == 0) {
      mbar_arrive_expect_tx(b_bar, num_kb * BOX);
      for (int kb = 0; kb < num_kb; ++kb) tma_load_3d(sb + kb * BOX, &tmB, b_bar, kb * GEMM_BK, tn * GEMM_BN, 0);
      uint32_t stage = 0, phase = 0;
      for (int tm = tm_start; tm < tiles_m; tm += tm_step) {
        for (int kb = 0; kb < num_kb; ++kb) {
          mbar_wait(&empty_bar[stage], phase ^ 1u);
          mbar_arrive_expect_tx(&full_bar[stage], BOX);
          tma_load_3d(sa + stage * BOX, &tmA, &full_bar[stage], kb * GEMM_BK, tm * GEMM_BM, 0);
          if (++stage == kStages) { stage = 0; phase ^= 1u; }
        }
      }
    }
  } else {
    warpgroup_reg_alloc<232>();
    const int mwg = wg - 1;
    constexpr uint32_t DESC_HI = smem_desc_hi_sw128(1024);
    constexpr uint32_t KSTEP = 32u >> 4;
    constexpr uint32_t A_HALF = 8192u >> 4;
    const uint32_t a_lo0 = smem_desc_lo(smem_u32(sa), 8192u);
    const uint32_t b_lo0 = smem_desc_lo(smem_u32(sb), 8192u);
    const bool leader = (threadIdx.x & 127) == 0;
    uint32_t stage = 0, phase = 0;
    float acc[2][GEMM_BN / 2];
    mbar_wait(b_bar, 0);
    int i = 0;
    for (int tm = tm_start; tm < tiles_m; tm += tm_step, ++i) {
      if ((i & 1) != mwg) {
        ring_advance<kStages>(stage, phase, num_kb);
        continue;
      }
      if (i > 0) mbar_wait(&turn_bar[mwg], ((i - 1) >> 1) & 1);
#pragma unroll
      for (int j = 0; j < GEMM_BN / 2; ++j) { acc[0][j] = 0.f; acc[1][j] = 0.f; }
      uint32_t prev_stage = 0;
      for (int kb = 0; kb < num_kb; ++kb) {
        mbar_wait(&full_bar[stage], phase);
        const uint32_t a_lo = a_lo0 + stage * (BOX >> 4);
        const uint32_t b_lo = b_lo0 + kb * (BOX >> 4);
        fence_operands(acc[0]);
        fence_operands(acc[1]);
        wgmma_fence();
#pragma unroll
        for (uint32_t k = 0; k < GEMM_BK / 16; ++k) {
          const uint64_t db = smem_desc_join(b_lo + k * KSTEP, DESC_HI);
#pragma unroll
          for (uint32_t h = 0; h < 2; ++h)
            wgmma_ss<GEMM_BN, 0, 0>(acc[h], smem_desc_join(a_lo + h * A_HALF + k * KSTEP, DESC_HI), db, 1u);
        }
        wgmma_commit();
        wgmma_wait<1>();
        if (kb > 0 && leader) mbar_arrive(&empty_bar[prev_stage]);
        prev_stage = stage;
        if (++stage == kStages) { stage = 0; phase ^= 1u; }
      }
      if (leader) mbar_arrive(&turn_bar[mwg ^ 1]);
      wgmma_wait<0>();
      fence_operands(acc[0]);
      fence_operands(acc[1]);
      if (leader) mbar_arrive(&empty_bar[prev_stage]);
      const int col_base = tn * GEMM_BN + 2 * (lane & 3);
      gemm_bias_act<GEMM_BN>(acc[0], p, col_base);
      gemm_bias_act<GEMM_BN>(acc[1], p, col_base);
      const uint32_t st = smem_u32(staging) + mwg * kBufs * GEMM_CHUNK_BYTES;
      if (p.out_bf16) gemm_store_tma<true, kBufs>(acc, p, &tmOut, st, 1 + mwg, leader, tm * GEMM_BM, tn * GEMM_BN, 0);
      else gemm_store_tma<false, kBufs>(acc, p, &tmOut, st, 1 + mwg, leader, tm * GEMM_BM, tn * GEMM_BN, 0);
    }
    if (leader) tma_wait_group<0>();
  }
}

template <int kStages, int kBufs>
static int launch_gemm_resident_kernel(const CUtensorMap& tmA, const CUtensorMap& tmB, const CUtensorMap& tmOut,
                                       const GemmParams& p, int grid, cudaStream_t stream) {
  constexpr size_t smem = GEMM_RES_B_BYTES + kStages * GEMM_RES_BOX_BYTES + 2 * kBufs * GEMM_CHUNK_BYTES + 1024 + 256;
  static_assert(smem <= 232448, "exceeds the 227 KB of shared memory a CTA can opt into");
  constexpr auto kern = gemm_bf16_resident_kernel<kStages, kBufs>;
  if (const int rc = opt_in_smem<kern>(smem, "gemm_bf16_resident_kernel"); rc != STEGO_OK) return rc;
  kern<<<grid, GEMM_THREADS, smem, stream>>>(tmA, tmB, tmOut, p);
  STEGO_CHECK_LAUNCH("gemm_bf16_resident_kernel launch");
  return STEGO_OK;
}

static int launch_gemm_resident(const CUtensorMap& tmA, const CUtensorMap& tmB, const CUtensorMap& tmOut,
                                const GemmParams& p, int grid, cudaStream_t stream) {
  if (p.act != 0) return launch_gemm_resident_kernel<6, 1>(tmA, tmB, tmOut, p, grid, stream);
  return launch_gemm_resident_kernel<4, 2>(tmA, tmB, tmOut, p, grid, stream);
}

}

using namespace stego;

static int gemm_impl(const void* A, int lda, long long a_bs, int a_mn_major, const void* B, int ldb, long long b_bs,
                     int b_mn_major, int batch, int M, int N, int K, void* out, int ldo, long long out_bs, int out_bf16,
                     const float* bias, int act, const float* residual, int ldr, long long res_bs, int row_div, int splits,
                     int atomic_out, cudaStream_t stream) {
  STEGO_CHECK_ARG(A && B && out, "stego_gemm_bf16: null pointer");
  STEGO_CHECK_ARG(M > 0 && N > 0 && K > 0 && batch > 0, "stego_gemm_bf16: bad sizes M=%d N=%d K=%d batch=%d", M, N, K, batch);
  STEGO_CHECK_ARG(lda % 8 == 0 && ldb % 8 == 0, "stego_gemm_bf16: lda/ldb must be multiples of 8 elements");
  STEGO_CHECK_ARG(batch == 1 || (a_bs % 8 == 0 && b_bs % 8 == 0 && row_div == 0),
                  "stego_gemm_bf16_batched: operand batch strides must be multiples of 8 elements");
  STEGO_CHECK_ARG(act >= 0 && act <= 2, "stego_gemm_bf16: act=%d", act);
  STEGO_CHECK_ARG(!(atomic_out && out_bf16), "stego_gemm_bf16: atomic output must be fp32");
  STEGO_CHECK_ARG(splits >= 1, "stego_gemm_bf16: splits=%d", splits);
  STEGO_CHECK_ARG(splits == 1 || atomic_out, "stego_gemm_bf16: split-K requires atomic_out");
  STEGO_CHECK_ARG(!atomic_out || (bias == nullptr && act == 0 && residual == nullptr),
                  "stego_gemm_bf16: atomic_out takes no bias, act or residual (bias=%p act=%d residual=%p)",
                  (const void*)bias, act, (const void*)residual);
  STEGO_CHECK_ARG(lda >= (a_mn_major ? M : K) && ldb >= (b_mn_major ? N : K),
                  "stego_gemm_bf16: lda=%d / ldb=%d shorter than a row (M=%d N=%d K=%d, a_mn_major=%d b_mn_major=%d)",
                  lda, ldb, M, N, K, a_mn_major, b_mn_major);
  STEGO_CHECK_ARG(ldo >= N && (residual == nullptr || ldr >= N),
                  "stego_gemm_bf16: ldo=%d / ldr=%d shorter than a row of N=%d", ldo, ldr, N);
  if (batch == 1) {
    a_bs = static_cast<long long>(a_mn_major ? K : M) * lda;
    b_bs = static_cast<long long>(b_mn_major ? K : N) * ldb;
    out_bs = static_cast<long long>(M) * ldo;
    res_bs = 0;
  }

  GemmParams p;
  p.M = M; p.N = N; p.K = K;
  const int num_kb = (K + GEMM_BK - 1) / GEMM_BK;
  if (splits > num_kb) splits = num_kb;
  p.kb_per_split = (num_kb + splits - 1) / splits;
  p.splits = (num_kb + p.kb_per_split - 1) / p.kb_per_split;
  p.out = out; p.ldo = ldo; p.out_bf16 = out_bf16;
  p.bias = bias; p.act = act;
  p.residual = residual; p.ldr = ldr;
  p.row_div = row_div; p.atomic = atomic_out;
  p.batch = batch; p.out_bs = out_bs; p.res_bs = res_bs;
  const size_t esz = out_bf16 ? 2 : 4;
  const size_t pair = 2 * esz;
  p.vec_ok = ((reinterpret_cast<uintptr_t>(out) % pair) == 0) && (ldo % 2 == 0) && (out_bs % 2 == 0) &&
             (residual == nullptr || ((reinterpret_cast<uintptr_t>(residual) % 8) == 0 && ldr % 2 == 0 && res_bs % 2 == 0)) &&
             (bias == nullptr || (reinterpret_cast<uintptr_t>(bias) % 8) == 0);
  const bool in_place = residual != nullptr && residual == out && ldr == ldo && !out_bf16;
  const bool tma_epi = !atomic_out && row_div == 0 && (residual == nullptr || in_place) &&
                       (reinterpret_cast<uintptr_t>(out) % 16) == 0 && (static_cast<size_t>(ldo) * esz) % 16 == 0 &&
                       (static_cast<size_t>(out_bs) * esz) % 16 == 0 && (static_cast<size_t>(N) * esz) % 16 == 0;
  p.reduce_add = tma_epi && in_place;

  CUtensorMap tmA, tmB, tmOut;
  int rc;
  {
    uint64_t dims[3] = {a_mn_major ? (uint64_t)M : (uint64_t)K, a_mn_major ? (uint64_t)K : (uint64_t)M, (uint64_t)batch};
    uint64_t str[2] = {(uint64_t)lda * 2, (uint64_t)a_bs * 2};
    uint32_t box[3] = {64, a_mn_major ? 64u : (uint32_t)GEMM_BM, 1};
    if ((rc = make_tmap_bf16(&tmA, A, 3, dims, str, box)) != STEGO_OK) return rc;
  }
  {
    uint64_t dims[3] = {b_mn_major ? (uint64_t)N : (uint64_t)K, b_mn_major ? (uint64_t)K : (uint64_t)N, (uint64_t)batch};
    uint64_t str[2] = {(uint64_t)ldb * 2, (uint64_t)b_bs * 2};
    uint32_t box[3] = {64, b_mn_major ? 64u : (uint32_t)GEMM_BN, 1};
    if ((rc = make_tmap_bf16(&tmB, B, 3, dims, str, box)) != STEGO_OK) return rc;
  }
  if (tma_epi) {
    uint64_t dims[3] = {(uint64_t)N, (uint64_t)M, (uint64_t)batch};
    uint64_t str[2] = {(uint64_t)ldo * esz, (uint64_t)out_bs * esz};
    uint32_t box[3] = {(uint32_t)(128 / esz), (uint32_t)GEMM_BM, 1};
    rc = out_bf16 ? make_tmap_bf16(&tmOut, out, 3, dims, str, box) : make_tmap_f32(&tmOut, out, 3, dims, str, box);
    if (rc != STEGO_OK) return rc;
  } else {
    memset(&tmOut, 0, sizeof(tmOut));
  }
  const int tiles_n = (N + GEMM_BN - 1) / GEMM_BN;
  const long long tiles = static_cast<long long>((M + GEMM_BM - 1) / GEMM_BM) * tiles_n;
  const int sms = num_sms();
  if (batch == 1 && !a_mn_major && !b_mn_major && tma_epi && K <= GEMM_RES_MAX_K && tiles >= 4LL * sms &&
      tiles_n <= sms)
    return launch_gemm_resident(tmA, tmB, tmOut, p, sms, stream);
  if (!a_mn_major && !b_mn_major) return launch_gemm_epi<false, false>(tma_epi, tmA, tmB, tmOut, p, stream);
  if (!a_mn_major && b_mn_major) return launch_gemm_epi<false, true>(tma_epi, tmA, tmB, tmOut, p, stream);
  if (a_mn_major && b_mn_major) return launch_gemm_epi<true, true>(tma_epi, tmA, tmB, tmOut, p, stream);
  return launch_gemm_epi<true, false>(tma_epi, tmA, tmB, tmOut, p, stream);
}

extern "C" int stego_gemm_bf16(const void* A, int lda, int a_mn_major, const void* B, int ldb, int b_mn_major, int M,
                               int N, int K, void* out, int ldo, int out_bf16, const float* bias, int act,
                               const float* residual, int ldr, int row_div, int splits, int atomic_out,
                               void* stream_) {
  return gemm_impl(A, lda, 0, a_mn_major, B, ldb, 0, b_mn_major, 1, M, N, K, out, ldo, 0, out_bf16, bias, act, residual, ldr, 0,
                   row_div, splits, atomic_out, reinterpret_cast<cudaStream_t>(stream_));
}

extern "C" int stego_gemm_bf16_batched(const void* A, int lda, long long a_batch_stride, int a_mn_major, const void* B,
                                       int ldb, long long b_batch_stride, int b_mn_major, int batch, int M, int N, int K,
                                       void* out, int ldo, long long out_batch_stride, int out_bf16, const float* bias,
                                       int act, void* stream_) {
  return gemm_impl(A, lda, a_batch_stride, a_mn_major, B, ldb, b_batch_stride, b_mn_major, batch, M, N, K, out, ldo,
                   out_batch_stride, out_bf16, bias, act, nullptr, 0, 0, 0, 1, 0, reinterpret_cast<cudaStream_t>(stream_));
}
```

stego_b200/csrc/host_util.cu:

```cuda
#include "host_util.h"

#include <atomic>
#include <stdarg.h>
#include <stdio.h>
#include <string.h>

namespace stego {

static thread_local char g_err[512] = "";

void set_error(const char* fmt, ...) {
  va_list ap;
  va_start(ap, fmt);
  vsnprintf(g_err, sizeof(g_err), fmt, ap);
  va_end(ap);
}

int cuda_fail(cudaError_t e, const char* what) {
  set_error("%s: %s (%s)", what, cudaGetErrorName(e), cudaGetErrorString(e));
  return STEGO_ERR_CUDA;
}

static std::atomic<long long> g_launches{0};
void count_launch() { g_launches.fetch_add(1, std::memory_order_relaxed); }
long long launch_count() { return g_launches.load(std::memory_order_relaxed); }

std::mutex& opt_in_mutex() {
  static std::mutex m;
  return m;
}

int num_sms() {
  static std::atomic<int> cached[kMaxCachedDevices];
  int dev = 0, n = 0;
  if (cudaGetDevice(&dev) != cudaSuccess) return 132;
  const bool cacheable = dev >= 0 && dev < kMaxCachedDevices;
  if (cacheable && (n = cached[dev].load(std::memory_order_relaxed)) > 0) return n;
  if (cudaDeviceGetAttribute(&n, cudaDevAttrMultiProcessorCount, dev) != cudaSuccess || n <= 0) return 132;
  if (cacheable) cached[dev].store(n, std::memory_order_relaxed);
  return n;
}

typedef CUresult (*EncodeTiledFn)(CUtensorMap*, CUtensorMapDataType, cuuint32_t, void*, const cuuint64_t*,
                                  const cuuint64_t*, const cuuint32_t*, const cuuint32_t*, CUtensorMapInterleave,
                                  CUtensorMapSwizzle, CUtensorMapL2promotion, CUtensorMapFloatOOBfill);

static EncodeTiledFn encode_fn() {
  static const EncodeTiledFn fn = []() -> EncodeTiledFn {
    void* p = nullptr;
    cudaDriverEntryPointQueryResult q;
    cudaError_t e = cudaGetDriverEntryPoint("cuTensorMapEncodeTiled", &p, cudaEnableDefault, &q);
    if (e != cudaSuccess || q != cudaDriverEntryPointSuccess || !p) return nullptr;
    return reinterpret_cast<EncodeTiledFn>(p);
  }();
  return fn;
}

static int make_tmap(CUtensorMapDataType dtype, CUtensorMap* out, const void* base, int rank, const uint64_t* dims,
                     const uint64_t* strides_bytes, const uint32_t* box) {
  EncodeTiledFn fn = encode_fn();
  if (!fn) {
    set_error("cuTensorMapEncodeTiled driver entry point unavailable");
    return STEGO_ERR_CUDA;
  }
  if (rank < 2 || rank > 3) {
    set_error("tensor map rank %d unsupported", rank);
    return STEGO_ERR_BAD_ARG;
  }
  if ((reinterpret_cast<uintptr_t>(base) & 15u) != 0) {
    set_error("tensor map base %p not 16-byte aligned", base);
    return STEGO_ERR_BAD_ARG;
  }
  cuuint64_t gdim[3];
  cuuint64_t gstr[2];
  cuuint32_t bdim[3];
  cuuint32_t estr[3] = {1, 1, 1};
  for (int i = 0; i < rank; ++i) {
    gdim[i] = dims[i];
    bdim[i] = box[i];
  }
  for (int i = 0; i < rank - 1; ++i) {
    if (strides_bytes[i] % 16 != 0) {
      set_error("tensor map stride %llu not a multiple of 16 bytes", (unsigned long long)strides_bytes[i]);
      return STEGO_ERR_BAD_ARG;
    }
    gstr[i] = strides_bytes[i];
  }
  CUresult r = fn(out, dtype, (cuuint32_t)rank, const_cast<void*>(base), gdim, gstr, bdim,
                  estr, CU_TENSOR_MAP_INTERLEAVE_NONE, CU_TENSOR_MAP_SWIZZLE_128B, CU_TENSOR_MAP_L2_PROMOTION_L2_256B,
                  CU_TENSOR_MAP_FLOAT_OOB_FILL_NONE);
  if (r != CUDA_SUCCESS) {
    set_error("cuTensorMapEncodeTiled failed with CUresult %d (rank %d dims %llu,%llu box %u,%u)", (int)r, rank,
              (unsigned long long)dims[0], (unsigned long long)dims[1], box[0], box[1]);
    return STEGO_ERR_CUDA;
  }
  return STEGO_OK;
}

int make_tmap_bf16(CUtensorMap* out, const void* base, int rank, const uint64_t* dims,
                   const uint64_t* strides_bytes, const uint32_t* box) {
  return make_tmap(CU_TENSOR_MAP_DATA_TYPE_BFLOAT16, out, base, rank, dims, strides_bytes, box);
}

int make_tmap_f32(CUtensorMap* out, const void* base, int rank, const uint64_t* dims,
                  const uint64_t* strides_bytes, const uint32_t* box) {
  return make_tmap(CU_TENSOR_MAP_DATA_TYPE_FLOAT32, out, base, rank, dims, strides_bytes, box);
}

}

extern "C" const char* stego_last_error(void) { return stego::g_err; }
extern "C" int stego_version(void) { return 100; }
extern "C" long long stego_launch_count(void) { return stego::launch_count(); }
```

stego_b200/csrc/host_util.h:

```cpp
#pragma once
#include <cuda.h>
#include <cuda_runtime.h>
#include <stdint.h>

#include <atomic>
#include <mutex>

namespace stego {

enum : int {
  STEGO_OK = 0,
  STEGO_ERR_BAD_ARG = -1,
  STEGO_ERR_UNSUPPORTED = -2,
  STEGO_ERR_CUDA = -3,
};

void set_error(const char* fmt, ...);
int cuda_fail(cudaError_t e, const char* what);
int num_sms();
void count_launch();

int make_tmap_bf16(CUtensorMap* out, const void* base, int rank, const uint64_t* dims,
                   const uint64_t* strides_bytes, const uint32_t* box);
int make_tmap_f32(CUtensorMap* out, const void* base, int rank, const uint64_t* dims,
                  const uint64_t* strides_bytes, const uint32_t* box);

constexpr int kMaxCachedDevices = 64;

std::mutex& opt_in_mutex();

template <auto Kernel>
int opt_in_smem(size_t bytes, const char* what) {
  static std::atomic<size_t> configured[kMaxCachedDevices];
  if (bytes <= 48 * 1024) return STEGO_OK;
  int dev = 0;
  cudaError_t e = cudaGetDevice(&dev);
  if (e != cudaSuccess) return cuda_fail(e, what);
  const bool cached = dev >= 0 && dev < kMaxCachedDevices;
  if (cached && configured[dev].load(std::memory_order_acquire) >= bytes) return STEGO_OK;
  std::lock_guard<std::mutex> lock(opt_in_mutex());
  if (cached && configured[dev].load(std::memory_order_relaxed) >= bytes) return STEGO_OK;
  e = cudaFuncSetAttribute(Kernel, cudaFuncAttributeMaxDynamicSharedMemorySize, (int)bytes);
  if (e != cudaSuccess) return cuda_fail(e, what);
  if (cached) configured[dev].store(bytes, std::memory_order_release);
  return STEGO_OK;
}

#define STEGO_CHECK_ARG(cond, ...)       \
  do {                                   \
    if (!(cond)) {                       \
      ::stego::set_error(__VA_ARGS__);   \
      return ::stego::STEGO_ERR_BAD_ARG; \
    }                                    \
  } while (0)

#define STEGO_CHECK_LAUNCH(what)                                     \
  do {                                                               \
    cudaError_t _e = cudaGetLastError();                             \
    if (_e != cudaSuccess) return ::stego::cuda_fail(_e, what);      \
    ::stego::count_launch();                                         \
  } while (0)

}
```

stego_b200/csrc/vit_misc.cu:

```cuda
#include "common.cuh"
#include "host_util.h"

namespace stego {

__device__ __forceinline__ uint32_t swap_bf16x2(uint32_t v) { return __byte_perm(v, 0, 0x1032); }

template <int P, typename T, bool MIRROR>
__global__ void patchify_kernel(const T* __restrict__ img, bf16* __restrict__ out, int B, int H, int W) {
  const int fh = H / P, fw = W / P;
  const long long total = 1ll * (MIRROR ? 2 * B : B) * fh * fw * 3 * P;
  const long long idx = 1ll * blockIdx.x * blockDim.x + threadIdx.x;
  if (idx >= total) return;
  const int ky = idx % P;
  const int c = (idx / P) % 3;
  const long long patch = idx / (3 * P);
  const int px = patch % fw;
  const int py = (patch / fw) % fh;
  const int b = patch / (1ll * fw * fh);
  const bool flip = MIRROR && b >= B;
  const int sb = flip ? b - B : b, sx = flip ? fw - 1 - px : px;
  const T* src = img + ((1ll * sb * 3 + c) * H + (py * P + ky)) * W + sx * P;
  bf16* dst = out + patch * (3 * P * P) + c * P * P + ky * P;
  static_assert(P == 8 || P == 16, "patch size");
#pragma unroll
  for (int v = 0; v < P / 8; ++v) {
    const int sv = flip ? P / 8 - 1 - v : v;
    uint4 w;
    if constexpr (sizeof(T) == 2) {
      w = *reinterpret_cast<const uint4*>(src + sv * 8);
    } else {
      const float4 a = *reinterpret_cast<const float4*>(src + sv * 8);
      const float4 b4 = *reinterpret_cast<const float4*>(src + sv * 8 + 4);
      w.x = pack_bf16x2(a.x, a.y);
      w.y = pack_bf16x2(a.z, a.w);
      w.z = pack_bf16x2(b4.x, b4.y);
      w.w = pack_bf16x2(b4.z, b4.w);
    }
    if (flip) w = make_uint4(swap_bf16x2(w.w), swap_bf16x2(w.z), swap_bf16x2(w.y), swap_bf16x2(w.x));
    *reinterpret_cast<uint4*>(dst + v * 8) = w;
  }
}

__global__ void cls_rows_kernel(float* __restrict__ x, const float* __restrict__ cls, const float* __restrict__ pos,
                                int B, int ntok, int E) {
  const int i = blockIdx.x * blockDim.x + threadIdx.x;
  if (i >= B * E) return;
  const int b = i / E, e = i % E;
  x[(1ll * b * ntok) * E + e] = cls[e] + pos[e];
}

template <int V4>
__global__ void __launch_bounds__(256)
layernorm_kernel(const float* __restrict__ x, const float* __restrict__ gamma, const float* __restrict__ beta,
                 bf16* __restrict__ out, int rows, float eps, int drop_cls) {
  constexpr int E = V4 * 128;
  const int row = blockIdx.x * (blockDim.x >> 5) + (threadIdx.x >> 5);
  if (row >= rows) return;
  const int lane = threadIdx.x & 31;
  long long orow = row;
  if (drop_cls > 0) {
    const int t = row % drop_cls;
    if (t == 0) return;
    orow = 1ll * (row / drop_cls) * (drop_cls - 1) + (t - 1);
  }
  const float4* xr = reinterpret_cast<const float4*>(x + 1ll * row * E);
  float4 v[V4];
  float s = 0.f;
#pragma unroll
  for (int i = 0; i < V4; ++i) {
    v[i] = xr[lane + 32 * i];
    s += (v[i].x + v[i].y) + (v[i].z + v[i].w);
  }
  const float mean = __fmul_rn(warp_sum(s), 1.0f / E);
  float q = 0.f;
#pragma unroll
  for (int i = 0; i < V4; ++i) {
    const float a = v[i].x - mean, b = v[i].y - mean, c = v[i].z - mean, d = v[i].w - mean;
    q += (a * a + b * b) + (c * c + d * d);
  }
  const float rstd = rsqrtf(warp_sum(q) * (1.0f / E) + eps);
  const float4* g4 = reinterpret_cast<const float4*>(gamma);
  const float4* b4 = reinterpret_cast<const float4*>(beta);
  uint2* o = reinterpret_cast<uint2*>(out + orow * E);
#pragma unroll
  for (int i = 0; i < V4; ++i) {
    const float4 g = __ldg(g4 + lane + 32 * i);
    const float4 bb = __ldg(b4 + lane + 32 * i);
    uint2 w;
    w.x = pack_bf16x2((v[i].x - mean) * rstd * g.x + bb.x, (v[i].y - mean) * rstd * g.y + bb.y);
    w.y = pack_bf16x2((v[i].z - mean) * rstd * g.z + bb.z, (v[i].w - mean) * rstd * g.w + bb.w);
    o[lane + 32 * i] = w;
  }
}

template <int V4>
__global__ void __launch_bounds__(256)
layernorm_gap_kernel(const float* __restrict__ x, const float* __restrict__ gamma, const float* __restrict__ beta,
                     float* __restrict__ out, int ntok, float eps, int rows_per_cta) {
  constexpr int E = V4 * 128;
  __shared__ float4 red[8][V4 * 32];
  const int b = blockIdx.y;
  const int warp = threadIdx.x >> 5, lane = threadIdx.x & 31;
  const int t0 = 1 + blockIdx.x * rows_per_cta;
  const int t1 = min(ntok, t0 + rows_per_cta);
  const float4* g4 = reinterpret_cast<const float4*>(gamma);
  float4 g[V4], acc[V4];
#pragma unroll
  for (int i = 0; i < V4; ++i) {
    g[i] = __ldg(g4 + lane + 32 * i);
    acc[i] = make_float4(0.f, 0.f, 0.f, 0.f);
  }
  int nrows = 0;
  for (int t = t0 + warp; t < t1; t += 8) {
    const float4* xr = reinterpret_cast<const float4*>(x + (1ll * b * ntok + t) * E);
    float4 v[V4];
    float s = 0.f;
#pragma unroll
    for (int i = 0; i < V4; ++i) {
      v[i] = xr[lane + 32 * i];
      s += (v[i].x + v[i].y) + (v[i].z + v[i].w);
    }
    const float mean = __fmul_rn(warp_sum(s), 1.0f / E);
    float q = 0.f;
#pragma unroll
    for (int i = 0; i < V4; ++i) {
      const float a = v[i].x - mean, bq = v[i].y - mean, c = v[i].z - mean, d = v[i].w - mean;
      q += (a * a + bq * bq) + (c * c + d * d);
    }
    const float rstd = rsqrtf(warp_sum(q) * (1.0f / E) + eps);
#pragma unroll
    for (int i = 0; i < V4; ++i) {
      acc[i].x += (v[i].x - mean) * rstd * g[i].x;
      acc[i].y += (v[i].y - mean) * rstd * g[i].y;
      acc[i].z += (v[i].z - mean) * rstd * g[i].z;
      acc[i].w += (v[i].w - mean) * rstd * g[i].w;
    }
    ++nrows;
  }
#pragma unroll
  for (int i = 0; i < V4; ++i) red[warp][lane + 32 * i] = acc[i];
  __shared__ int cnt[8];
  if (lane == 0) cnt[warp] = nrows;
  __syncthreads();
  const float inv = 1.0f / (ntok - 1);
  int total = 0;
#pragma unroll
  for (int w = 0; w < 8; ++w) total += cnt[w];
  for (int c4 = threadIdx.x; c4 < V4 * 32; c4 += blockDim.x) {
    float4 sum = make_float4(0.f, 0.f, 0.f, 0.f);
#pragma unroll
    for (int w = 0; w < 8; ++w) {
      const float4 r = red[w][c4];
      sum.x += r.x; sum.y += r.y; sum.z += r.z; sum.w += r.w;
    }
    const float4 bb = __ldg(reinterpret_cast<const float4*>(beta) + c4);
    float* o = out + 1ll * b * E + 4 * c4;
    atomicAdd(o + 0, (sum.x + total * bb.x) * inv);
    atomicAdd(o + 1, (sum.y + total * bb.y) * inv);
    atomicAdd(o + 2, (sum.z + total * bb.z) * inv);
    atomicAdd(o + 3, (sum.w + total * bb.w) * inv);
  }
}

__global__ void __launch_bounds__(256)
linear_rows_f32_kernel(const float* __restrict__ x, const bf16* __restrict__ w, int ldw, const float* __restrict__ bias,
                       float* __restrict__ out, int B, int N, int K) {
  const long long o = 1ll * blockIdx.x * (blockDim.x >> 5) + (threadIdx.x >> 5);
  if (o >= 1ll * B * N) return;
  const int lane = threadIdx.x & 31;
  const int b = static_cast<int>(o / N), n = static_cast<int>(o % N);
  const float4* xr = reinterpret_cast<const float4*>(x + 1ll * b * K);
  const uint4* wr = reinterpret_cast<const uint4*>(w + 1ll * n * ldw);
  float acc = 0.f;
  for (int c = lane; c < K / 8; c += 32) {
    const uint4 wv = __ldg(wr + c);
    const float4 x0 = __ldg(xr + 2 * c), x1 = __ldg(xr + 2 * c + 1);
    const bf16* wb = reinterpret_cast<const bf16*>(&wv);
    acc = fmaf(x0.x, __bfloat162float(wb[0]), acc);
    acc = fmaf(x0.y, __bfloat162float(wb[1]), acc);
    acc = fmaf(x0.z, __bfloat162float(wb[2]), acc);
    acc = fmaf(x0.w, __bfloat162float(wb[3]), acc);
    acc = fmaf(x1.x, __bfloat162float(wb[4]), acc);
    acc = fmaf(x1.y, __bfloat162float(wb[5]), acc);
    acc = fmaf(x1.z, __bfloat162float(wb[6]), acc);
    acc = fmaf(x1.w, __bfloat162float(wb[7]), acc);
  }
  acc = warp_sum(acc);
  if (lane == 0) out[o] = acc + (bias ? bias[n] : 0.f);
}

}

using namespace stego;

template <bool MIRROR>
static int launch_patchify(const void* img, int img_is_bf16, void* out_bf16, int B, int H, int W, int patch,
                           cudaStream_t stream) {
  const char* name = MIRROR ? "stego_vit_patchify_tta" : "stego_vit_patchify";
  STEGO_CHECK_ARG(img && out_bf16, "%s: null pointer", name);
  STEGO_CHECK_ARG(patch == 8 || patch == 16, "%s: patch size %d unsupported (8 or 16)", name, patch);
  STEGO_CHECK_ARG(B > 0 && H % patch == 0 && W % patch == 0 && W % 8 == 0, "%s: bad image %dx%dx%d", name, B, H, W);
  STEGO_CHECK_ARG((reinterpret_cast<uintptr_t>(img) & 15u) == 0, "%s: image not 16-byte aligned", name);
  const long long total = 1ll * (MIRROR ? 2 * B : B) * (H / patch) * (W / patch) * 3 * patch;
  const int threads = 256;
  const int blocks = (int)((total + threads - 1) / threads);
  bf16* out = reinterpret_cast<bf16*>(out_bf16);
  if (img_is_bf16) {
    const bf16* im = reinterpret_cast<const bf16*>(img);
    if (patch == 8) patchify_kernel<8, bf16, MIRROR><<<blocks, threads, 0, stream>>>(im, out, B, H, W);
    else patchify_kernel<16, bf16, MIRROR><<<blocks, threads, 0, stream>>>(im, out, B, H, W);
  } else {
    const float* im = reinterpret_cast<const float*>(img);
    if (patch == 8) patchify_kernel<8, float, MIRROR><<<blocks, threads, 0, stream>>>(im, out, B, H, W);
    else patchify_kernel<16, float, MIRROR><<<blocks, threads, 0, stream>>>(im, out, B, H, W);
  }
  STEGO_CHECK_LAUNCH("patchify_kernel");
  return STEGO_OK;
}

extern "C" int stego_vit_patchify(const float* img, void* out_bf16, int B, int H, int W, int patch, void* stream_) {
  return launch_patchify<false>(img, 0, out_bf16, B, H, W, patch, reinterpret_cast<cudaStream_t>(stream_));
}

extern "C" int stego_vit_patchify_bf16(const void* img_bf16, void* out_bf16, int B, int H, int W, int patch,
                                       void* stream_) {
  return launch_patchify<false>(img_bf16, 1, out_bf16, B, H, W, patch, reinterpret_cast<cudaStream_t>(stream_));
}

extern "C" int stego_vit_patchify_tta(const void* img, int img_is_bf16, void* out_bf16, int B, int H, int W, int patch,
                                      void* stream_) {
  return launch_patchify<true>(img, img_is_bf16, out_bf16, B, H, W, patch, reinterpret_cast<cudaStream_t>(stream_));
}

extern "C" int stego_vit_cls_rows(float* x, const float* cls_token, const float* pos_embed, int B, int ntok, int E,
                                  void* stream_) {
  cudaStream_t stream = reinterpret_cast<cudaStream_t>(stream_);
  STEGO_CHECK_ARG(x && cls_token && pos_embed && B > 0 && ntok > 0 && E > 0, "stego_vit_cls_rows: bad args");
  cls_rows_kernel<<<(B * E + 255) / 256, 256, 0, stream>>>(x, cls_token, pos_embed, B, ntok, E);
  STEGO_CHECK_LAUNCH("cls_rows_kernel");
  return STEGO_OK;
}

extern "C" int stego_layernorm_bf16(const float* x, const float* gamma, const float* beta, void* out_bf16, int rows,
                                    int E, float eps, int drop_cls_ntok, void* stream_) {
  cudaStream_t stream = reinterpret_cast<cudaStream_t>(stream_);
  STEGO_CHECK_ARG(x && gamma && beta && out_bf16 && rows > 0, "stego_layernorm_bf16: bad args");
  STEGO_CHECK_ARG(drop_cls_ntok == 0 || rows % drop_cls_ntok == 0, "stego_layernorm_bf16: rows %% ntok != 0");
  const int warps = 8;
  const int blocks = (rows + warps - 1) / warps;
  bf16* o = reinterpret_cast<bf16*>(out_bf16);
  switch (E) {
    case 384: layernorm_kernel<3><<<blocks, warps * 32, 0, stream>>>(x, gamma, beta, o, rows, eps, drop_cls_ntok); break;
    case 768: layernorm_kernel<6><<<blocks, warps * 32, 0, stream>>>(x, gamma, beta, o, rows, eps, drop_cls_ntok); break;
    case 128: layernorm_kernel<1><<<blocks, warps * 32, 0, stream>>>(x, gamma, beta, o, rows, eps, drop_cls_ntok); break;
    case 192:
    default:
      set_error("stego_layernorm_bf16: embed dim %d unsupported (128, 384, 768)", E);
      return STEGO_ERR_UNSUPPORTED;
  }
  STEGO_CHECK_LAUNCH("layernorm_kernel");
  return STEGO_OK;
}

extern "C" int stego_layernorm_gap(const float* x, const float* gamma, const float* beta, float* out, int B, int ntok,
                                   int E, float eps, void* stream_) {
  cudaStream_t stream = reinterpret_cast<cudaStream_t>(stream_);
  STEGO_CHECK_ARG(x && gamma && beta && out && B > 0 && ntok > 1, "stego_layernorm_gap: bad args");
  const int rows_per_cta = 64;
  dim3 grid((ntok - 1 + rows_per_cta - 1) / rows_per_cta, B);
  switch (E) {
    case 384: layernorm_gap_kernel<3><<<grid, 256, 0, stream>>>(x, gamma, beta, out, ntok, eps, rows_per_cta); break;
    case 768: layernorm_gap_kernel<6><<<grid, 256, 0, stream>>>(x, gamma, beta, out, ntok, eps, rows_per_cta); break;
    case 128: layernorm_gap_kernel<1><<<grid, 256, 0, stream>>>(x, gamma, beta, out, ntok, eps, rows_per_cta); break;
    default:
      set_error("stego_layernorm_gap: embed dim %d unsupported (128, 384, 768)", E);
      return STEGO_ERR_UNSUPPORTED;
  }
  STEGO_CHECK_LAUNCH("layernorm_gap_kernel");
  return STEGO_OK;
}

extern "C" int stego_linear_rows_f32(const float* x, const void* w_bf16, int ldw, const float* bias, float* out, int B,
                                     int N, int K, void* stream_) {
  cudaStream_t stream = reinterpret_cast<cudaStream_t>(stream_);
  STEGO_CHECK_ARG(x && w_bf16 && out, "stego_linear_rows_f32: null pointer");
  STEGO_CHECK_ARG(B > 0 && N > 0 && K > 0 && K % 8 == 0, "stego_linear_rows_f32: bad sizes B=%d N=%d K=%d (K a multiple of 8)",
                  B, N, K);
  STEGO_CHECK_ARG(ldw >= K && ldw % 8 == 0, "stego_linear_rows_f32: ldw=%d (>= K, a multiple of 8)", ldw);
  STEGO_CHECK_ARG((reinterpret_cast<uintptr_t>(x) & 15u) == 0 && (reinterpret_cast<uintptr_t>(w_bf16) & 15u) == 0,
                  "stego_linear_rows_f32: x and w must be 16-byte aligned");
  const long long outputs = 1ll * B * N;
  const int warps = 8;
  const long long blocks = (outputs + warps - 1) / warps;
  STEGO_CHECK_ARG(blocks <= 0x7fffffffll, "stego_linear_rows_f32: B*N=%lld too large", outputs);
  linear_rows_f32_kernel<<<static_cast<unsigned>(blocks), warps * 32, 0, stream>>>(
      x, reinterpret_cast<const bf16*>(w_bf16), ldw, bias, out, B, N, K);
  STEGO_CHECK_LAUNCH("linear_rows_f32_kernel");
  return STEGO_OK;
}
```

stego_b200/dino/vision_transformer.py:

```python
from __future__ import annotations

import math
import threading
from functools import partial
from typing import Dict, List, Optional, Tuple

import torch
import torch.nn as nn

from .. import ops

_PREPARE_LOCK = threading.RLock()


def _to_device(w, dev):
    if isinstance(w, dict):
        return {k: _to_device(v, dev) for k, v in w.items()}
    if isinstance(w, list):
        return [_to_device(v, dev) for v in w]
    return w.to(dev) if isinstance(w, torch.Tensor) else w


class Mlp(nn.Module):

    def __init__(self, in_features, hidden_features=None, out_features=None, act_layer=nn.GELU, drop=0.):
        super().__init__()
        self.fc1 = nn.Linear(in_features, hidden_features or in_features)
        self.act = act_layer()
        self.fc2 = nn.Linear(hidden_features or in_features, out_features or in_features)
        self.drop = nn.Dropout(drop)


class Attention(nn.Module):

    def __init__(self, dim, num_heads=8, qkv_bias=False, qk_scale=None, attn_drop=0., proj_drop=0.):
        super().__init__()
        self.num_heads = num_heads
        self.scale = qk_scale or (dim // num_heads) ** -0.5
        self.qkv = nn.Linear(dim, dim * 3, bias=qkv_bias)
        self.attn_drop = nn.Dropout(attn_drop)
        self.proj = nn.Linear(dim, dim)
        self.proj_drop = nn.Dropout(proj_drop)


class Block(nn.Module):

    def __init__(self, dim, num_heads, mlp_ratio=4., qkv_bias=False, qk_scale=None, drop=0., attn_drop=0.,
                 drop_path=0., act_layer=nn.GELU, norm_layer=nn.LayerNorm):
        super().__init__()
        self.norm1 = norm_layer(dim)
        self.attn = Attention(dim, num_heads=num_heads, qkv_bias=qkv_bias, qk_scale=qk_scale, attn_drop=attn_drop,
                              proj_drop=drop)
        self.drop_path = nn.Identity()
        self.norm2 = norm_layer(dim)
        self.mlp = Mlp(in_features=dim, hidden_features=int(dim * mlp_ratio), act_layer=act_layer, drop=drop)


class PatchEmbed(nn.Module):

    def __init__(self, img_size=224, patch_size=16, in_chans=3, embed_dim=768):
        super().__init__()
        self.img_size = img_size
        self.patch_size = patch_size
        self.num_patches = (img_size // patch_size) * (img_size // patch_size)
        self.proj = nn.Conv2d(in_chans, embed_dim, kernel_size=patch_size, stride=patch_size)


class VisionTransformer(nn.Module):

    def __init__(self, img_size=[224], patch_size=16, in_chans=3, num_classes=0, embed_dim=768, depth=12,
                 num_heads=12, mlp_ratio=4., qkv_bias=False, qk_scale=None, drop_rate=0., attn_drop_rate=0.,
                 drop_path_rate=0., norm_layer=nn.LayerNorm, **kwargs):
        super().__init__()
        if in_chans != 3:
            raise ValueError("stego_b200 ViT: in_chans must be 3")
        if embed_dim % num_heads != 0 or embed_dim // num_heads != 64:
            raise ValueError("stego_b200 ViT: head_dim must be 64 (vit_small / vit_base)")
        self.num_features = self.embed_dim = embed_dim
        self.num_heads = num_heads
        self.mlp_ratio = mlp_ratio
        self.patch_embed = PatchEmbed(img_size=img_size[0], patch_size=patch_size, in_chans=in_chans,
                                      embed_dim=embed_dim)
        self.cls_token = nn.Parameter(torch.zeros(1, 1, embed_dim))
        self.pos_embed = nn.Parameter(torch.zeros(1, self.patch_embed.num_patches + 1, embed_dim))
        self.pos_drop = nn.Dropout(p=drop_rate)
        self.blocks = nn.ModuleList([
            Block(dim=embed_dim, num_heads=num_heads, mlp_ratio=mlp_ratio, qkv_bias=qkv_bias, qk_scale=qk_scale,
                  drop=drop_rate, attn_drop=attn_drop_rate, norm_layer=norm_layer) for _ in range(depth)])
        self.norm = norm_layer(embed_dim)
        self.head = nn.Linear(embed_dim, num_classes) if num_classes > 0 else nn.Identity()
        nn.init.trunc_normal_(self.pos_embed, std=.02)
        nn.init.trunc_normal_(self.cls_token, std=.02)
        self.apply(self._init_weights)
        self._cache: Dict[str, object] = {}

    @staticmethod
    def _init_weights(m):
        if isinstance(m, nn.Linear):
            nn.init.trunc_normal_(m.weight, std=.02)
            if m.bias is not None:
                nn.init.constant_(m.bias, 0)
        elif isinstance(m, nn.LayerNorm):
            nn.init.constant_(m.bias, 0)
            nn.init.constant_(m.weight, 1.0)

    def _weights_key(self):
        return tuple((p.data_ptr(), p._version) for p in self.parameters())

    def _replicate_for_data_parallel(self):
        replica = super()._replicate_for_data_parallel()
        replica.__dict__["_master"] = self._root()
        return replica

    def _root(self) -> "VisionTransformer":
        return self.__dict__.get("_master", self)

    def _prepared(self, device=None):
        master = self._root()
        home = master.cls_token.device
        dev = home if device is None else torch.device(device)
        with _PREPARE_LOCK:
            key = master._weights_key()
            if master._cache.get("key") != key:
                master._cache = {"key": key, "w": {}, "pos": {}}
            ws = master._cache["w"]
            if home not in ws:
                ws[home] = master._prepare_weights(home)
            if dev not in ws:
                ws[dev] = _to_device(ws[home], dev)
            return ws[dev]

    def _prepare_weights(self, dev):
        E = self.embed_dim
        w = {}
        w["pe_w"] = self.patch_embed.proj.weight.detach().reshape(E, -1).to(torch.bfloat16).contiguous()
        w["pe_b"] = self.patch_embed.proj.bias.detach().float().contiguous()
        w["cls"] = self.cls_token.detach().float().reshape(E).contiguous()
        blocks = []
        for blk in self.blocks:
            def f32(t, n):
                return t.detach().float().contiguous() if t is not None else torch.zeros(n, device=dev)
            blocks.append(dict(
                n1w=f32(blk.norm1.weight, E), n1b=f32(blk.norm1.bias, E), eps1=blk.norm1.eps,
                qkv_w=blk.attn.qkv.weight.detach().to(torch.bfloat16).contiguous(),
                qkv_b=f32(blk.attn.qkv.bias, 3 * E),
                proj_w=blk.attn.proj.weight.detach().to(torch.bfloat16).contiguous(),
                proj_b=f32(blk.attn.proj.bias, E),
                n2w=f32(blk.norm2.weight, E), n2b=f32(blk.norm2.bias, E), eps2=blk.norm2.eps,
                fc1_w=blk.mlp.fc1.weight.detach().to(torch.bfloat16).contiguous(), fc1_b=f32(blk.mlp.fc1.bias, blk.mlp.fc1.out_features),
                fc2_w=blk.mlp.fc2.weight.detach().to(torch.bfloat16).contiguous(), fc2_b=f32(blk.mlp.fc2.bias, E)))
        w["blocks"] = blocks
        w["nw"] = self.norm.weight.detach().float().contiguous()
        w["nb"] = self.norm.bias.detach().float().contiguous()
        return w

    def interpolate_pos_encoding(self, x, w, h):
        npatch = x.shape[1] - 1
        N = self.pos_embed.shape[1] - 1
        if npatch == N and w == h:
            return self.pos_embed
        dim = x.shape[-1]
        p = self.patch_embed.patch_size
        w0, h0 = w // p + 0.1, h // p + 0.1
        side = int(math.sqrt(N))
        grid = self.pos_embed[:, 1:].reshape(1, side, side, dim).permute(0, 3, 1, 2)
        grid = nn.functional.interpolate(grid, scale_factor=(w0 / math.sqrt(N), h0 / math.sqrt(N)), mode='bicubic')
        assert int(w0) == grid.shape[-2] and int(h0) == grid.shape[-1]
        grid = grid.permute(0, 2, 3, 1).reshape(1, -1, dim)
        return torch.cat((self.pos_embed[:, :1], grid), dim=1)

    def _pos_for(self, H: int, W: int, device=None) -> torch.Tensor:
        master = self._root()
        home = master.cls_token.device
        dev = home if device is None else torch.device(device)
        self._prepared(dev)
        with _PREPARE_LOCK:
            cache = master._cache["pos"]
            if (H, W, home) not in cache:
                p = master.patch_embed.patch_size
                ntok = (H // p) * (W // p) + 1
                with torch.no_grad():
                    dummy = torch.empty(1, ntok, master.embed_dim, device="meta")
                    pos = master.interpolate_pos_encoding(dummy, H, W)
                cache[(H, W, home)] = pos.detach().float().reshape(ntok, master.embed_dim).contiguous()
            if (H, W, dev) not in cache:
                cache[(H, W, dev)] = cache[(H, W, home)].to(dev)
            return cache[(H, W, dev)]

    @torch.no_grad()
    def forward_tokens(self, img: torch.Tensor, want_qkv: bool = False, taps: Optional["BlockTaps"] = None,
                       stop_before_last: bool = False, mirror: bool = False
                       ) -> Tuple[torch.Tensor, Optional[torch.Tensor]]:
        if not img.is_cuda:
            raise RuntimeError("stego_b200: the DINO ViT forward only exists as sm_90a kernels (no CPU fallback)")
        w = self._prepared(img.device)
        img = (img if img.dtype == torch.bfloat16 else img.float()).contiguous()
        B, _, H, W = img.shape
        B = 2 * B if mirror else B
        p = self.patch_embed.patch_size
        E, heads = self.embed_dim, self.num_heads
        hw = (H // p) * (W // p)
        N = hw + 1
        dev = img.device
        pos = self._pos_for(H, W, dev)
        rows = ops.patchify_tta(img, p) if mirror else ops.patchify(img, p)
        x = torch.empty(B * N, E, dtype=torch.float32, device=dev)
        ops.gemm(rows, w["pe_w"], x, M=B * hw, N=E, K=3 * p * p, bias=w["pe_b"], residual=pos, row_div=hw)
        ops.cls_rows(x, w["cls"], pos, B, N)
        y = torch.empty(B * N, E, dtype=torch.bfloat16, device=dev)
        qkv = torch.empty(B * N, 3 * E, dtype=torch.bfloat16, device=dev)
        ao = torch.empty(B * N, E, dtype=torch.bfloat16, device=dev)
        hid = torch.empty(B * N, w["blocks"][0]["fc1_w"].shape[0], dtype=torch.bfloat16, device=dev)
        Hd = hid.shape[1]
        blocks = w["blocks"]
        depth = len(blocks)
        for i, bw in enumerate(blocks[:-1] if stop_before_last else blocks):
            tap = taps is not None and depth - i <= taps.n
            ops.layernorm(x, bw["n1w"], bw["n1b"], y, eps=bw["eps1"])
            ops.gemm(y, bw["qkv_w"], qkv, M=B * N, N=3 * E, K=E, bias=bw["qkv_b"])
            if tap:
                taps.qkv.append(qkv.clone())
                if taps.probs:
                    taps.attn.append(ops.attention_probs(
                        qkv, torch.empty(B, heads, N, N, dtype=torch.float32, device=dev), B, N, E, heads))
                if taps.stop_at_last_probs and i == depth - 1:
                    break
            ops.attention(qkv, ao, B, N, E, heads)
            ops.gemm(ao, bw["proj_w"], x, M=B * N, N=E, K=E, bias=bw["proj_b"], residual=x)
            ops.layernorm(x, bw["n2w"], bw["n2b"], y, eps=bw["eps2"])
            ops.gemm(y, bw["fc1_w"], hid, M=B * N, N=Hd, K=E, bias=bw["fc1_b"], act=ops.ACT_GELU)
            ops.gemm(hid, bw["fc2_w"], x, M=B * N, N=E, K=Hd, bias=bw["fc2_b"], residual=x)
            if tap:
                taps.x.append(x.clone())
        return x, (qkv if want_qkv else None)

    @torch.no_grad()
    def patch_features(self, img: torch.Tensor, use_graph: bool = False, mirror: bool = False) -> torch.Tensor:
        return self._tokens(img, use_graph, "feat", mirror)

    @torch.no_grad()
    def key_features(self, img: torch.Tensor, use_graph: bool = False, mirror: bool = False) -> torch.Tensor:
        return self._tokens(img, use_graph, "KK", mirror)

    def _tokens(self, img, use_graph: bool, kind: str, mirror: bool = False) -> torch.Tensor:
        kind = kind + "+mirror" if mirror else kind
        if use_graph and (img[0] if isinstance(img, (list, tuple)) else img).is_cuda:
            return self._graphed(img, kind)
        if isinstance(img, (list, tuple)):
            img = torch.cat(list(img), 0)
        return self._eager(img, kind)

    def _eager(self, img: torch.Tensor, kind: str) -> torch.Tensor:
        mirror = kind.endswith("+mirror")
        if kind.startswith("feat"):
            return self._patch_features_eager(img, mirror)
        return self._key_features_eager(img, mirror)

    def _graphed(self, img, kind: str) -> torch.Tensor:
        from .. import _lib
        parts = list(img) if isinstance(img, (list, tuple)) else [img]
        self._prepared(parts[0].device)
        graphs = self._root()._cache.setdefault("graphs", {})
        shape = (sum(p.shape[0] for p in parts),) + tuple(parts[0].shape[1:])
        dt = torch.bfloat16 if all(p.dtype == torch.bfloat16 for p in parts) else torch.float32
        key = (kind, shape, parts[0].device.index, dt)
        if key not in graphs:
            img = torch.cat([p.to(dt) for p in parts], 0) if len(parts) > 1 else parts[0].to(dt)
            self._eager(img, kind)
            static_in = img.detach().contiguous().clone()
            with torch.cuda.device(static_in.device):
                graphs[key] = (_lib.Graph(lambda: self._eager(static_in, kind)), static_in)
        g, static_in = graphs[key]
        off = 0
        for part in parts:
            if part.data_ptr() != static_in[off].data_ptr():
                static_in[off:off + part.shape[0]].copy_(part)
            off += part.shape[0]
        g.replay()
        return g.result

    def graph_input(self, kind: str, shape, device, dtype=torch.float32):
        return self._root()._cache.get("graphs", {}).get((kind, tuple(shape), device.index, dtype), (None, None))[1]

    def _patch_features_eager(self, img: torch.Tensor, mirror: bool = False) -> torch.Tensor:
        B = img.shape[0] * (2 if mirror else 1)
        x, _ = self.forward_tokens(img, mirror=mirror)
        w = self._prepared(x.device)
        N = x.shape[0] // B
        out = torch.empty(B * (N - 1), self.embed_dim, dtype=torch.bfloat16, device=x.device)
        ops.layernorm(x, w["nw"], w["nb"], out, eps=self.norm.eps, drop_cls_ntok=N)
        return out.view(B, N - 1, self.embed_dim)

    def _key_features_eager(self, img: torch.Tensor, mirror: bool = False) -> torch.Tensor:
        B, E = img.shape[0] * (2 if mirror else 1), self.embed_dim
        x, _ = self.forward_tokens(img, stop_before_last=True, mirror=mirror)
        bw = self._prepared(x.device)["blocks"][-1]
        N = x.shape[0] // B
        y = torch.empty(B * (N - 1), E, dtype=torch.bfloat16, device=x.device)
        ops.layernorm(x, bw["n1w"], bw["n1b"], y, eps=bw["eps1"], drop_cls_ntok=N)
        out = torch.empty(B * (N - 1), E, dtype=torch.bfloat16, device=x.device)
        ops.gemm(y, bw["qkv_w"][E:2 * E], out, M=B * (N - 1), N=E, K=E, bias=bw["qkv_b"][E:2 * E])
        return out.view(B, N - 1, E)

    @torch.no_grad()
    def pooled_patch_features(self, img: torch.Tensor) -> torch.Tensor:
        from .. import _lib
        B = img.shape[0]
        x, _ = self.forward_tokens(img)
        w = self._prepared(x.device)
        out = torch.zeros(B, self.embed_dim, dtype=torch.float32, device=x.device)
        _lib.check(_lib.load().stego_layernorm_gap(_lib.ptr(x), _lib.ptr(w["nw"]), _lib.ptr(w["nb"]), _lib.ptr(out), B,
                                                   x.shape[0] // B, self.embed_dim, float(self.norm.eps), _lib.stream()),
                   "stego_layernorm_gap")
        return out

    @torch.no_grad()
    def pooled_key_features(self, img: torch.Tensor) -> torch.Tensor:
        from .. import _lib
        B, E = img.shape[0], self.embed_dim
        x, _ = self.forward_tokens(img, stop_before_last=True)
        bw = self._prepared(x.device)["blocks"][-1]
        pooled = torch.zeros(B, E, dtype=torch.float32, device=x.device)
        lib = _lib.load()
        _lib.check(lib.stego_layernorm_gap(_lib.ptr(x), _lib.ptr(bw["n1w"]), _lib.ptr(bw["n1b"]), _lib.ptr(pooled), B,
                                           x.shape[0] // B, E, float(bw["eps1"]), _lib.stream()), "stego_layernorm_gap")
        return ops.linear_rows_f32(pooled, bw["qkv_w"][E:2 * E], bw["qkv_b"][E:2 * E])

    def _all_tokens(self, img: torch.Tensor, want_qkv: bool = False):
        x, qkv = self.forward_tokens(img, want_qkv)
        return self.final_norm(x, img.shape[0]), qkv

    def forward(self, x):
        tok, _ = self._all_tokens(x)
        return tok[:, 0].float()

    def forward_feats(self, x):
        tok, _ = self._all_tokens(x)
        return tok.float()

    def block_taps(self, img: torch.Tensor, n: int, probs: bool = False, stop_at_last_probs: bool = False
                   ) -> "BlockTaps":
        taps = BlockTaps(min(n, len(self.blocks)), probs, stop_at_last_probs)
        self.forward_tokens(img, taps=taps)
        return taps

    def final_norm(self, x: torch.Tensor, B: int) -> torch.Tensor:
        w = self._prepared(x.device)
        out = torch.empty(x.shape[0], self.embed_dim, dtype=torch.bfloat16, device=x.device)
        ops.layernorm(x, w["nw"], w["nb"], out, eps=self.norm.eps)
        return out.view(B, -1, self.embed_dim)

    def split_qkv(self, qkv: torch.Tensor, B: int) -> torch.Tensor:
        E = self.embed_dim
        return qkv.view(B, -1, 3, self.num_heads, E // self.num_heads).permute(2, 0, 3, 1, 4).float()

    def get_intermediate_feat(self, x, n=1):
        if n <= 0:
            return [], [], []
        B = x.shape[0]
        taps = self.block_taps(x, n, probs=True)
        return ([self.final_norm(t, B).float() for t in taps.x], taps.attn,
                [self.split_qkv(q, B) for q in taps.qkv])

    def get_last_selfattention(self, x):
        return self.block_taps(x, 1, probs=True, stop_at_last_probs=True).attn[0]

    def get_intermediate_layers(self, x, n=1):
        if n <= 0:
            return []
        B = x.shape[0]
        return [self.final_norm(t, B).float() for t in self.block_taps(x, n).x]


class BlockTaps:

    def __init__(self, n: int, probs: bool = False, stop_at_last_probs: bool = False):
        self.n, self.probs, self.stop_at_last_probs = n, probs, stop_at_last_probs
        self.qkv: List[torch.Tensor] = []
        self.attn: List[torch.Tensor] = []
        self.x: List[torch.Tensor] = []


def vit_tiny(patch_size=16, **kwargs):
    raise ValueError("stego_b200: vit_tiny (head_dim 64, embed 192) is not built for this path")


def vit_small(patch_size=16, **kwargs):
    return VisionTransformer(patch_size=patch_size, embed_dim=384, depth=12, num_heads=6, mlp_ratio=4,
                             qkv_bias=True, norm_layer=partial(nn.LayerNorm, eps=1e-6), **kwargs)


def vit_base(patch_size=16, **kwargs):
    return VisionTransformer(patch_size=patch_size, embed_dim=768, depth=12, num_heads=12, mlp_ratio=4,
                             qkv_bias=True, norm_layer=partial(nn.LayerNorm, eps=1e-6), **kwargs)
```

stego_b200/ops.py:

```python
from __future__ import annotations

from typing import Optional

import torch

from . import _lib

ACT_NONE, ACT_GELU, ACT_RELU = 0, 1, 2


def gemm(a: torch.Tensor, b: torch.Tensor, out: torch.Tensor, *, M: int, N: int, K: int,
         a_mn: bool = False, b_mn: bool = False, bias: Optional[torch.Tensor] = None, act: int = ACT_NONE,
         residual: Optional[torch.Tensor] = None, row_div: int = 0, splits: int = 1,
         atomic: bool = False) -> torch.Tensor:
    _lib.require_cuda(a, b, out, bias, residual)
    assert a.dtype == torch.bfloat16 and b.dtype == torch.bfloat16
    assert a.dim() == 2 and b.dim() == 2 and out.dim() == 2
    assert a.stride(1) == 1 and b.stride(1) == 1 and out.stride(1) == 1
    assert out.dtype in (torch.bfloat16, torch.float32)
    if bias is not None:
        assert bias.dtype == torch.float32 and bias.is_contiguous()
    if residual is not None:
        assert residual.dtype == torch.float32 and residual.stride(1) == 1
    rc = _lib.load().stego_gemm_bf16(
        _lib.ptr(a), a.stride(0), int(a_mn), _lib.ptr(b), b.stride(0), int(b_mn), M, N, K,
        _lib.ptr(out), out.stride(0), int(out.dtype == torch.bfloat16), _lib.ptr(bias), act,
        _lib.ptr(residual), residual.stride(0) if residual is not None else 0, row_div, splits, int(atomic),
        _lib.stream())
    _lib.check(rc, "stego_gemm_bf16")
    return out


def wgrad_splits(K: int, out_rows: int, out_cols: int, num_sms: int) -> int:
    tiles = ((out_rows + 127) // 128) * ((out_cols + 127) // 128)
    return max(1, min(K // 512, num_sms // tiles))


def gemm_batched(a: torch.Tensor, b: torch.Tensor, out: torch.Tensor, *, a_mn: bool = False, b_mn: bool = False,
                 bias: Optional[torch.Tensor] = None, act: int = ACT_NONE) -> torch.Tensor:
    _lib.require_cuda(a, b, out, bias)
    assert a.dtype == torch.bfloat16 and b.dtype == torch.bfloat16 and a.dim() == 3 and b.dim() == 3 and out.dim() == 3
    assert a.stride(2) == 1 and b.stride(2) == 1 and out.stride(2) == 1 and out.dtype in (torch.bfloat16, torch.float32)
    n = a.shape[0]
    M, K = (a.shape[2], a.shape[1]) if a_mn else (a.shape[1], a.shape[2])
    N = b.shape[2] if b_mn else b.shape[1]
    assert b.shape[0] == n and out.shape == (n, M, N) and (b.shape[1] if b_mn else b.shape[2]) == K
    rc = _lib.load().stego_gemm_bf16_batched(
        _lib.ptr(a), a.stride(1), a.stride(0), int(a_mn), _lib.ptr(b), b.stride(1), b.stride(0), int(b_mn), n, M, N, K,
        _lib.ptr(out), out.stride(1), out.stride(0), int(out.dtype == torch.bfloat16), _lib.ptr(bias), act, _lib.stream())
    _lib.check(rc, "stego_gemm_bf16_batched")
    return out


def patchify(img: torch.Tensor, patch: int) -> torch.Tensor:
    _lib.require_cuda(img)
    assert img.dtype in (torch.float32, torch.bfloat16) and img.is_contiguous() and img.shape[1] == 3
    B, _, H, W = img.shape
    out = torch.empty(B * (H // patch) * (W // patch), 3 * patch * patch, dtype=torch.bfloat16, device=img.device)
    lib = _lib.load()
    fn = lib.stego_vit_patchify if img.dtype == torch.float32 else lib.stego_vit_patchify_bf16
    _lib.check(fn(_lib.ptr(img), _lib.ptr(out), B, H, W, patch, _lib.stream()), "stego_vit_patchify")
    return out


def patchify_tta(img: torch.Tensor, patch: int) -> torch.Tensor:
    _lib.require_cuda(img)
    assert img.dtype in (torch.float32, torch.bfloat16) and img.is_contiguous() and img.shape[1] == 3
    B, _, H, W = img.shape
    out = torch.empty(2 * B * (H // patch) * (W // patch), 3 * patch * patch, dtype=torch.bfloat16, device=img.device)
    _lib.check(_lib.load().stego_vit_patchify_tta(_lib.ptr(img), int(img.dtype == torch.bfloat16), _lib.ptr(out), B, H, W,
                                                  patch, _lib.stream()), "stego_vit_patchify_tta")
    return out


def cls_rows(x: torch.Tensor, cls_token: torch.Tensor, pos_embed: torch.Tensor, B: int, ntok: int) -> None:
    E = x.shape[-1]
    _lib.check(_lib.load().stego_vit_cls_rows(_lib.ptr(x), _lib.ptr(cls_token), _lib.ptr(pos_embed), B, ntok, E,
                                              _lib.stream()), "stego_vit_cls_rows")


def layernorm(x: torch.Tensor, gamma: torch.Tensor, beta: torch.Tensor, out: torch.Tensor, eps: float = 1e-6,
              drop_cls_ntok: int = 0) -> torch.Tensor:
    _lib.require_cuda(x, gamma, beta, out)
    assert x.dtype == torch.float32 and x.is_contiguous() and out.dtype == torch.bfloat16 and out.is_contiguous()
    rows, E = x.shape
    _lib.check(_lib.load().stego_layernorm_bf16(_lib.ptr(x), _lib.ptr(gamma), _lib.ptr(beta), _lib.ptr(out), rows, E,
                                                eps, drop_cls_ntok, _lib.stream()), "stego_layernorm_bf16")
    return out


def linear_rows_f32(x: torch.Tensor, w: torch.Tensor, bias: Optional[torch.Tensor] = None) -> torch.Tensor:
    _lib.require_cuda(x, w, bias)
    assert x.dtype == torch.float32 and x.dim() == 2 and x.is_contiguous()
    assert w.dtype == torch.bfloat16 and w.dim() == 2 and w.stride(1) == 1 and w.shape[1] == x.shape[1]
    if bias is not None:
        assert bias.dtype == torch.float32 and bias.is_contiguous() and bias.numel() == w.shape[0]
    B, K = x.shape
    N = w.shape[0]
    out = torch.empty(B, N, dtype=torch.float32, device=x.device)
    _lib.check(_lib.load().stego_linear_rows_f32(_lib.ptr(x), _lib.ptr(w), w.stride(0), _lib.ptr(bias), _lib.ptr(out),
                                                 B, N, K, _lib.stream()), "stego_linear_rows_f32")
    return out


def attention(qkv: torch.Tensor, out: torch.Tensor, B: int, N: int, E: int, heads: int) -> torch.Tensor:
    _lib.require_cuda(qkv, out)
    assert qkv.dtype == torch.bfloat16 and qkv.is_contiguous() and out.dtype == torch.bfloat16 and out.is_contiguous()
    _lib.check(_lib.load().stego_attention_fwd(_lib.ptr(qkv), _lib.ptr(out), B, N, E, heads, _lib.stream()),
               "stego_attention_fwd")
    return out


def attention_probs(qkv: torch.Tensor, out: torch.Tensor, B: int, N: int, E: int, heads: int) -> torch.Tensor:
    _lib.require_cuda(qkv, out)
    assert qkv.dtype == torch.bfloat16 and qkv.is_contiguous() and qkv.shape == (B * N, 3 * E)
    assert out.dtype == torch.float32 and out.is_contiguous() and out.numel() == B * heads * N * N
    _lib.check(_lib.load().stego_attention_probs(_lib.ptr(qkv), _lib.ptr(out), B, N, E, heads, _lib.stream()),
               "stego_attention_probs")
    return out


LABEL_BYTES = {torch.int64: 8, torch.int32: 4, torch.uint8: 1}


def probe_label(label: torch.Tensor, B: int, H: int, W: int):
    lab = label.reshape(B, H, W)
    if lab.dtype not in LABEL_BYTES:
        lab = lab.to(torch.long)
    lab = lab.contiguous()
    return lab, LABEL_BYTES[lab.dtype]


def tokens_major(code: torch.Tensor) -> torch.Tensor:
    x = code.detach()
    B, _, h, w = x.shape
    if (x.dtype != torch.float32 or x.stride(1) != 1 or x.stride(2) != w * x.stride(3)
            or (B > 1 and x.stride(0) != h * w * x.stride(3))):
        x = x.float().permute(0, 2, 3, 1).contiguous().permute(0, 3, 1, 2)
    return x


def probe_scratch(device) -> torch.Tensor:
    sms = torch.cuda.get_device_properties(device).multi_processor_count
    return torch.empty(16 * sms, dtype=torch.float32, device=device)
```

Baseline: 3089.

## Enable programmatic dependent launch across ViT kernels with frozen-weight prefetch

Launches GEMM, attention, layernorm, patchify and cls kernels with programmatic stream serialization and adds griddepcontrol wait/trigger points, so each kernel's prologue can overlap the previous kernel's tail inside the CUDA graph. For frozen backbone weights, the resident GEMM issues its B-operand TMA loads before waiting on the predecessor. Attention also skips the idle second consumer warpgroup on partial query tiles. PDL is on by default and can be turned off with an env var. Risks include ordering hazards if a trigger fires before all dependent writes are visible, and the assumption that B is not written by the preceding kernel.

After: 3138, median of 6. 1.6% higher.

```diff
diff --git a/include/stego_b200.h b/include/stego_b200.h
--- a/include/stego_b200.h
+++ b/include/stego_b200.h
@@ -10,11 +10,17 @@
 STEGO_API int stego_version(void);
 STEGO_API const char* stego_last_error(void);
 STEGO_API long long stego_launch_count(void);
+STEGO_API int stego_set_pdl(int on);
+STEGO_API int stego_pdl_enabled(void);
 
 STEGO_API int stego_gemm_bf16(const void* A, int lda, int a_mn_major, const void* B, int ldb, int b_mn_major,
                               int M, int N, int K, void* out, int ldo, int out_bf16, const float* bias, int act,
                               const float* residual, int ldr, int row_div, int splits, int atomic_out,
                               void* stream);
+STEGO_API int stego_gemm_bf16_frozen_b(const void* A, int lda, int a_mn_major, const void* B, int ldb, int b_mn_major,
+                                       int M, int N, int K, void* out, int ldo, int out_bf16, const float* bias,
+                                       int act, const float* residual, int ldr, int row_div, int splits,
+                                       int atomic_out, void* stream);
 
 STEGO_API int stego_gemm_bf16_batched(const void* A, int lda, long long a_batch_stride, int a_mn_major, const void* B,
                                       int ldb, long long b_batch_stride, int b_mn_major, int batch, int M, int N, int K,
diff --git a/profiles/pdl_time.py b/profiles/pdl_time.py
--- /dev/null
+++ b/profiles/pdl_time.py
@@ -0,0 +1,117 @@
+import argparse
+import os
+import statistics
+import sys
+import time
+
+import torch
+
+ROOT = os.path.dirname(os.path.dirname(os.path.abspath(__file__)))
+sys.path.insert(0, ROOT)
+sys.path.insert(0, os.path.join(ROOT, "oracle"))
+from _measure import card, emit, window_ms
+
+N_CLASSES = 27
+SHAPES = {"c1": ("vit_small", 224, 32), "c2": ("vit_base", 320, 32)}
+
+
+def _graphs(name, dev):
+    import stego_oracle as O
+    from stego_b200.config import make_cfg
+    from stego_b200.segmenter import LitUnsupervisedSegmenter
+    arch, res, B = SHAPES[name]
+    g = torch.Generator().manual_seed(1)
+    batch = dict(img=torch.randn(B, 3, res, res, generator=g).to(dev),
+                 img_pos=torch.randn(B, 3, res, res, generator=g).to(dev),
+                 label=torch.randint(-1, N_CLASSES, (B, res, res), generator=g).to(dev))
+    torch.manual_seed(0)
+    m = LitUnsupervisedSegmenter(N_CLASSES, make_cfg(model_type=arch, random_backbone_init=True)).to(dev)
+    m.net.model.load_state_dict(O.perturb_vit_state(O.vit_random_state(arch, 8, seed=3)))
+    m.train()
+    m.configure_optimizers()
+    for s in range(3):
+        m.training_step(batch, s)
+    m.flush()
+    torch.cuda.synchronize()
+    vit_graphs = list(m.net.model._root()._cache["graphs"].values())
+    assert len(vit_graphs) == 1 and m._fused.ws.graph is not None, name
+    return m, {"backbone": vit_graphs[0][0], "tail": m._fused.ws.graph[0]}
+
+
+def _trace(graph, replays):
+    from torch.profiler import ProfilerActivity, profile
+    graph.replay()
+    torch.cuda.synchronize()
+    with profile(activities=[ProfilerActivity.CUDA]) as prof:
+        for _ in range(replays):
+            graph.replay()
+            torch.cuda.synchronize()
+            time.sleep(0.005)
+    spans = sorted((e.time_range.start, e.time_range.end) for e in prof.events()
+                   if e.device_type == torch.autograd.DeviceType.CUDA and e.time_range.end > e.time_range.start
+                   and "memcpy" not in e.name.lower() and "memset" not in e.name.lower())
+    groups, cur = [], []
+    for s in spans:
+        if cur and s[0] - max(e for _, e in cur) > 1000.0:
+            groups.append(cur)
+            cur = []
+        cur.append(s)
+    if cur:
+        groups.append(cur)
+    assert len(groups) == replays, (len(groups), replays)
+    return groups
+
+
+def _boundaries(groups):
+    rows = []
+    for spans in groups:
+        busy = sum(e - s for s, e in spans)
+        wall = max(e for _, e in spans) - spans[0][0]
+        gaps = [spans[i + 1][0] - spans[i][1] for i in range(len(spans) - 1)]
+        rows.append(dict(kernels=len(spans), kernel_sum_us=busy, wall_us=wall, idle_us=wall - busy,
+                         gap_median_us=statistics.median(gaps) if gaps else 0.0, gap_max_us=max(gaps) if gaps else 0.0))
+    med = {k: statistics.median(r[k] for r in rows) for k in rows[0]}
+    med["kernels"] = int(med["kernels"])
+    return {k: (round(v, 2) if isinstance(v, float) else v) for k, v in med.items()}
+
+
+def main():
+    ap = argparse.ArgumentParser()
+    ap.add_argument("--pdl", default="both", choices=["on", "off", "both"])
+    ap.add_argument("--configs", default="c1,c2")
+    ap.add_argument("--trace-replays", type=int, default=5)
+    ap.add_argument("--out", default=None)
+    args = ap.parse_args()
+    from stego_b200 import _lib
+    dev = torch.device("cuda:0")
+    torch.cuda.set_device(dev)
+    settings = {"on": [True], "off": [False], "both": [False, True]}[args.pdl]
+    result = {"card": card(), "what": __doc__.split("\n\n")[0].replace("\n", " "), "configs": {}}
+    was = _lib.set_pdl(True)
+    try:
+        for name in args.configs.split(","):
+            arch, res, B = SHAPES[name]
+            per = {}
+            for on in settings:
+                _lib.set_pdl(on)
+                model, graphs = _graphs(name, dev)
+                entry = {}
+                for gname, graph in graphs.items():
+                    ms, n = window_ms(graph.replay, warmup=10, min_window_s=1.0, min_iters=50)
+                    entry[gname] = dict(replay_ms=round(ms, 4), replays_timed=n,
+                                        trace=_boundaries(_trace(graph, args.trace_replays)))
+                per["on" if on else "off"] = entry
+                del model, graphs
+                torch.cuda.synchronize()
+                torch.cuda.empty_cache()
+            if len(per) == 2:
+                per["saved_ms"] = {g: round(per["off"][g]["replay_ms"] - per["on"][g]["replay_ms"], 4)
+                                   for g in per["off"]}
+            result["configs"][name] = dict(arch=arch, res=res, batch=B, **per)
+    finally:
+        _lib.set_pdl(was)
+    emit(result, args.out, indent=1)
+
+
+if __name__ == "__main__":
+    main()
diff --git a/stego_b200/_lib.py b/stego_b200/_lib.py
--- a/stego_b200/_lib.py
+++ b/stego_b200/_lib.py
@@ -77,6 +77,14 @@
     return int(load().stego_launch_count()) + replayed_launches
 
 
+def pdl_enabled() -> bool:
+    return bool(load().stego_pdl_enabled())
+
+
+def set_pdl(on: bool) -> bool:
+    return bool(load().stego_set_pdl(int(bool(on))))
+
+
 _CAPTURE_LOCK = threading.Lock()
 
 
diff --git a/stego_b200/csrc/attention.cu b/stego_b200/csrc/attention.cu
--- a/stego_b200/csrc/attention.cu
+++ b/stego_b200/csrc/attention.cu
@@ -39,12 +39,13 @@
   const int head = blockIdx.y;
   const int img = blockIdx.z;
   const int nkv = (p.N + ATT_BKV - 1) / ATT_BKV;
+  const int live_wgs = q0 + 64 < p.N ? 2 : 1;
 
   if (threadIdx.x == 0) {
     mbar_init(q_full, 1);
     for (int s = 0; s < ATT_STAGES; ++s) {
       mbar_init(&kv_full[s], 1);
-      mbar_init(&kv_empty[s], 2);
+      mbar_init(&kv_empty[s], live_wgs);
     }
     fence_barrier_init();
   }
@@ -54,6 +55,7 @@
     if (lane == 0) {
       tma_prefetch_desc(&tmQKV);
       tma_prefetch_desc(&tmOut);
+      pdl_wait();
       mbar_arrive_expect_tx(q_full, ATT_Q_BYTES);
       tma_load_3d(smem + ATT_SMEM_Q, &tmQKV, q_full, head * ATT_D, q0, img);
       tma_load_3d(smem + ATT_SMEM_Q + ATT_Q_BYTES / 2, &tmQKV, q_full, head * ATT_D, q0 + 64, img);
@@ -66,11 +68,14 @@
         tma_load_3d(sk + ATT_KV_BYTES, &tmQKV, &kv_full[stage], 2 * p.E + head * ATT_D, j * ATT_BKV, img);
         if (++stage == ATT_STAGES) { stage = 0; phase ^= 1u; }
       }
+      pdl_trigger();
     }
     return;
   }
 
   const int wg = warp >> 2;
+  if (wg >= live_wgs) return;
+  pdl_wait();
   const int wq = warp & 3;
   const bool leader = (threadIdx.x & 127) == 0;
   const float c = p.scale_log2e;
@@ -336,9 +341,7 @@
   p.E = E;
   p.scale_log2e = 0.125f * 1.4426950408889634f;
   dim3 grid((N + ATT_BQ - 1) / ATT_BQ, heads, B);
-  attention_fwd_kernel<<<grid, ATT_THREADS, ATT_SMEM_TOTAL, stream>>>(tm, tmo, p);
-  STEGO_CHECK_LAUNCH("attention_fwd_kernel");
-  return STEGO_OK;
+  return launch_pdl("attention_fwd_kernel", attention_fwd_kernel, grid, ATT_THREADS, ATT_SMEM_TOTAL, stream, tm, tmo, p);
 }
 
 extern "C" int stego_attention_probs(const void* qkv, float* probs, int B, int N, int E, int heads, void* stream_) {
diff --git a/stego_b200/csrc/common.cuh b/stego_b200/csrc/common.cuh
--- a/stego_b200/csrc/common.cuh
+++ b/stego_b200/csrc/common.cuh
@@ -89,6 +89,9 @@
     }
   }
 }
+
+__device__ __forceinline__ void pdl_wait() { asm volatile("griddepcontrol.wait;\n" ::: "memory"); }
+__device__ __forceinline__ void pdl_trigger() { asm volatile("griddepcontrol.launch_dependents;\n" ::: "memory"); }
 
 __device__ __forceinline__ void tma_prefetch_desc(const CUtensorMap* m) {
   asm volatile("prefetch.tensormap [%0];\n" ::"l"(reinterpret_cast<uint64_t>(m)) : "memory");
diff --git a/stego_b200/csrc/gemm.cu b/stego_b200/csrc/gemm.cu
--- a/stego_b200/csrc/gemm.cu
+++ b/stego_b200/csrc/gemm.cu
@@ -32,6 +32,7 @@
   int batch;
   long long out_bs;
   long long res_bs;
+  int b_frozen;
 };
 
 template <int BN>
@@ -224,6 +225,7 @@
   if (wg == 0) {
     warpgroup_reg_dealloc<40>();
     if (threadIdx.x == 0) {
+      pdl_wait();
       uint32_t stage = 0, phase = 0;
       for (int t = sched_start; t < total_tiles; t += sched_step) {
         const int tb = t / tiles_per_batch, tl = t % tiles_per_batch;
@@ -254,9 +256,11 @@
           if (++stage == kStages) { stage = 0; phase ^= 1u; }
         }
       }
+      pdl_trigger();
     }
   } else {
     warpgroup_reg_alloc<232>();
+    pdl_wait();
     const int mwg = wg - 1;
     constexpr uint32_t DESC_HI = smem_desc_hi_sw128(1024);
     constexpr uint32_t A_KSTEP = A_MN ? (2048u >> 4) : (32u >> 4);
@@ -338,9 +342,7 @@
   const int tiles_n = (p.N + GEMM_BN - 1) / GEMM_BN;
   const int tiles = tiles_m * tiles_n * p.splits * p.batch;
   const int grid = tiles < num_sms() ? tiles : num_sms();
-  kern<<<grid, GEMM_THREADS, smem, stream>>>(tmA, tmB, tmOut, p);
-  STEGO_CHECK_LAUNCH("gemm_bf16_kernel launch");
-  return STEGO_OK;
+  return launch_pdl("gemm_bf16_kernel launch", kern, grid, GEMM_THREADS, smem, stream, tmA, tmB, tmOut, p);
 }
 
 template <bool A_MN, bool B_MN>
@@ -399,8 +401,10 @@
   if (wg == 0) {
     warpgroup_reg_dealloc<40>();
     if (threadIdx.x == 0) {
+      if (!p.b_frozen) pdl_wait();
       mbar_arrive_expect_tx(b_bar, num_kb * BOX);
       for (int kb = 0; kb < num_kb; ++kb) tma_load_3d(sb + kb * BOX, &tmB, b_bar, kb * GEMM_BK, tn * GEMM_BN, 0);
+      if (p.b_frozen) pdl_wait();
       uint32_t stage = 0, phase = 0;
       for (int tm = tm_start; tm < tiles_m; tm += tm_step) {
         for (int kb = 0; kb < num_kb; ++kb) {
@@ -410,9 +414,11 @@
           if (++stage == kStages) { stage = 0; phase ^= 1u; }
         }
       }
+      pdl_trigger();
     }
   } else {
     warpgroup_reg_alloc<232>();
+    pdl_wait();
     const int mwg = wg - 1;
     constexpr uint32_t DESC_HI = smem_desc_hi_sw128(1024);
     constexpr uint32_t KSTEP = 32u >> 4;
@@ -476,9 +482,7 @@
   static_assert(smem <= 232448, "exceeds the 227 KB of shared memory a CTA can opt into");
   constexpr auto kern = gemm_bf16_resident_kernel<kStages, kBufs>;
   if (const int rc = opt_in_smem<kern>(smem, "gemm_bf16_resident_kernel"); rc != STEGO_OK) return rc;
-  kern<<<grid, GEMM_THREADS, smem, stream>>>(tmA, tmB, tmOut, p);
-  STEGO_CHECK_LAUNCH("gemm_bf16_resident_kernel launch");
-  return STEGO_OK;
+  return launch_pdl("gemm_bf16_resident_kernel launch", kern, grid, GEMM_THREADS, smem, stream, tmA, tmB, tmOut, p);
 }
 
 static int launch_gemm_resident(const CUtensorMap& tmA, const CUtensorMap& tmB, const CUtensorMap& tmOut,
@@ -494,7 +498,7 @@
 static int gemm_impl(const void* A, int lda, long long a_bs, int a_mn_major, const void* B, int ldb, long long b_bs,
                      int b_mn_major, int batch, int M, int N, int K, void* out, int ldo, long long out_bs, int out_bf16,
                      const float* bias, int act, const float* residual, int ldr, long long res_bs, int row_div, int splits,
-                     int atomic_out, cudaStream_t stream) {
+                     int atomic_out, int b_frozen, cudaStream_t stream) {
   STEGO_CHECK_ARG(A && B && out, "stego_gemm_bf16: null pointer");
   STEGO_CHECK_ARG(M > 0 && N > 0 && K > 0 && batch > 0, "stego_gemm_bf16: bad sizes M=%d N=%d K=%d batch=%d", M, N, K, batch);
   STEGO_CHECK_ARG(lda % 8 == 0 && ldb % 8 == 0, "stego_gemm_bf16: lda/ldb must be multiples of 8 elements");
@@ -530,6 +534,7 @@
   p.residual = residual; p.ldr = ldr;
   p.row_div = row_div; p.atomic = atomic_out;
   p.batch = batch; p.out_bs = out_bs; p.res_bs = res_bs;
+  p.b_frozen = b_frozen;
   const size_t esz = out_bf16 ? 2 : 4;
   const size_t pair = 2 * esz;
   p.vec_ok = ((reinterpret_cast<uintptr_t>(out) % pair) == 0) && (ldo % 2 == 0) && (out_bs % 2 == 0) &&
@@ -581,7 +586,15 @@
                                const float* residual, int ldr, int row_div, int splits, int atomic_out,
                                void* stream_) {
   return gemm_impl(A, lda, 0, a_mn_major, B, ldb, 0, b_mn_major, 1, M, N, K, out, ldo, 0, out_bf16, bias, act, residual, ldr, 0,
-                   row_div, splits, atomic_out, reinterpret_cast<cudaStream_t>(stream_));
+                   row_div, splits, atomic_out, 0, reinterpret_cast<cudaStream_t>(stream_));
+}
+
+extern "C" int stego_gemm_bf16_frozen_b(const void* A, int lda, int a_mn_major, const void* B, int ldb, int b_mn_major,
+                                        int M, int N, int K, void* out, int ldo, int out_bf16, const float* bias,
+                                        int act, const float* residual, int ldr, int row_div, int splits,
+                                        int atomic_out, void* stream_) {
+  return gemm_impl(A, lda, 0, a_mn_major, B, ldb, 0, b_mn_major, 1, M, N, K, out, ldo, 0, out_bf16, bias, act, residual, ldr, 0,
+                   row_div, splits, atomic_out, 1, reinterpret_cast<cudaStream_t>(stream_));
 }
 
 extern "C" int stego_gemm_bf16_batched(const void* A, int lda, long long a_batch_stride, int a_mn_major, const void* B,
@@ -589,5 +602,5 @@
                                        void* out, int ldo, long long out_batch_stride, int out_bf16, const float* bias,
                                        int act, void* stream_) {
   return gemm_impl(A, lda, a_batch_stride, a_mn_major, B, ldb, b_batch_stride, b_mn_major, batch, M, N, K, out, ldo,
-                   out_batch_stride, out_bf16, bias, act, nullptr, 0, 0, 0, 1, 0, reinterpret_cast<cudaStream_t>(stream_));
-}
+                   out_batch_stride, out_bf16, bias, act, nullptr, 0, 0, 0, 1, 0, 0, reinterpret_cast<cudaStream_t>(stream_));
+}
diff --git a/stego_b200/csrc/host_util.cu b/stego_b200/csrc/host_util.cu
--- a/stego_b200/csrc/host_util.cu
+++ b/stego_b200/csrc/host_util.cu
@@ -2,6 +2,7 @@
 
 #include <atomic>
 #include <stdarg.h>
+#include <stdlib.h>
 #include <stdio.h>
 #include <string.h>
 
@@ -24,6 +25,24 @@
 static std::atomic<long long> g_launches{0};
 void count_launch() { g_launches.fetch_add(1, std::memory_order_relaxed); }
 long long launch_count() { return g_launches.load(std::memory_order_relaxed); }
+
+static std::atomic<int> g_pdl{-1};
+bool pdl_enabled() {
+  int v = g_pdl.load(std::memory_order_relaxed);
+  if (v < 0) {
+    const char* env = getenv("STEGO_PDL");
+    v = (env != nullptr && strcmp(env, "0") == 0) ? 0 : 1;
+    int unread = -1;
+    g_pdl.compare_exchange_strong(unread, v, std::memory_order_relaxed);
+    v = g_pdl.load(std::memory_order_relaxed);
+  }
+  return v != 0;
+}
+bool set_pdl(bool on) {
+  const bool was = pdl_enabled();
+  g_pdl.store(on ? 1 : 0, std::memory_order_relaxed);
+  return was;
+}
 
 std::mutex& opt_in_mutex() {
   static std::mutex m;
@@ -112,3 +131,5 @@
 extern "C" const char* stego_last_error(void) { return stego::g_err; }
 extern "C" int stego_version(void) { return 100; }
 extern "C" long long stego_launch_count(void) { return stego::launch_count(); }
+extern "C" int stego_set_pdl(int on) { return stego::set_pdl(on != 0) ? 1 : 0; }
+extern "C" int stego_pdl_enabled(void) { return stego::pdl_enabled() ? 1 : 0; }
diff --git a/stego_b200/csrc/host_util.h b/stego_b200/csrc/host_util.h
--- a/stego_b200/csrc/host_util.h
+++ b/stego_b200/csrc/host_util.h
@@ -5,6 +5,7 @@
 
 #include <atomic>
 #include <mutex>
+#include <utility>
 
 namespace stego {
 
@@ -61,4 +62,28 @@
     ::stego::count_launch();                                         \
   } while (0)
 
+bool pdl_enabled();
+bool set_pdl(bool on);
+
+template <typename... KArgs, typename... Args>
+int launch_pdl(const char* what, void (*kern)(KArgs...), dim3 grid, dim3 block, size_t smem, cudaStream_t stream,
+               Args&&... args) {
+  cudaLaunchAttribute attr[1];
+  attr[0].id = cudaLaunchAttributeProgrammaticStreamSerialization;
+  attr[0].val.programmaticStreamSerializationAllowed = 1;
+  cudaLaunchConfig_t cfg = {};
+  cfg.gridDim = grid;
+  cfg.blockDim = block;
+  cfg.dynamicSmemBytes = smem;
+  cfg.stream = stream;
+  cfg.attrs = attr;
+  cfg.numAttrs = pdl_enabled() ? 1 : 0;
+  cudaError_t e = cudaLaunchKernelEx(&cfg, kern, std::forward<Args>(args)...);
+  const cudaError_t last = cudaGetLastError();
+  if (e == cudaSuccess) e = last;
+  if (e != cudaSuccess) return cuda_fail(e, what);
+  count_launch();
+  return STEGO_OK;
 }
+
+}
diff --git a/stego_b200/csrc/vit_misc.cu b/stego_b200/csrc/vit_misc.cu
--- a/stego_b200/csrc/vit_misc.cu
+++ b/stego_b200/csrc/vit_misc.cu
@@ -7,6 +7,7 @@
 
 template <int P, typename T, bool MIRROR>
 __global__ void patchify_kernel(const T* __restrict__ img, bf16* __restrict__ out, int B, int H, int W) {
+  pdl_wait();
   const int fh = H / P, fw = W / P;
   const long long total = 1ll * (MIRROR ? 2 * B : B) * fh * fw * 3 * P;
   const long long idx = 1ll * blockIdx.x * blockDim.x + threadIdx.x;
@@ -39,14 +40,17 @@
     if (flip) w = make_uint4(swap_bf16x2(w.w), swap_bf16x2(w.z), swap_bf16x2(w.y), swap_bf16x2(w.x));
     *reinterpret_cast<uint4*>(dst + v * 8) = w;
   }
+  pdl_trigger();
 }
 
 __global__ void cls_rows_kernel(float* __restrict__ x, const float* __restrict__ cls, const float* __restrict__ pos,
                                 int B, int ntok, int E) {
+  pdl_wait();
   const int i = blockIdx.x * blockDim.x + threadIdx.x;
   if (i >= B * E) return;
   const int b = i / E, e = i % E;
   x[(1ll * b * ntok) * E + e] = cls[e] + pos[e];
+  pdl_trigger();
 }
 
 template <int V4>
@@ -54,6 +58,7 @@
 layernorm_kernel(const float* __restrict__ x, const float* __restrict__ gamma, const float* __restrict__ beta,
                  bf16* __restrict__ out, int rows, float eps, int drop_cls) {
   constexpr int E = V4 * 128;
+  pdl_wait();
   const int row = blockIdx.x * (blockDim.x >> 5) + (threadIdx.x >> 5);
   if (row >= rows) return;
   const int lane = threadIdx.x & 31;
@@ -91,6 +96,7 @@
     w.y = pack_bf16x2((v[i].z - mean) * rstd * g.z + bb.z, (v[i].w - mean) * rstd * g.w + bb.w);
     o[lane + 32 * i] = w;
   }
+  pdl_trigger();
 }
 
 template <int V4>
@@ -207,15 +213,12 @@
   bf16* out = reinterpret_cast<bf16*>(out_bf16);
   if (img_is_bf16) {
     const bf16* im = reinterpret_cast<const bf16*>(img);
-    if (patch == 8) patchify_kernel<8, bf16, MIRROR><<<blocks, threads, 0, stream>>>(im, out, B, H, W);
-    else patchify_kernel<16, bf16, MIRROR><<<blocks, threads, 0, stream>>>(im, out, B, H, W);
-  } else {
-    const float* im = reinterpret_cast<const float*>(img);
-    if (patch == 8) patchify_kernel<8, float, MIRROR><<<blocks, threads, 0, stream>>>(im, out, B, H, W);
-    else patchify_kernel<16, float, MIRROR><<<blocks, threads, 0, stream>>>(im, out, B, H, W);
-  }
-  STEGO_CHECK_LAUNCH("patchify_kernel");
-  return STEGO_OK;
+    const auto kern = patch == 8 ? patchify_kernel<8, bf16, MIRROR> : patchify_kernel<16, bf16, MIRROR>;
+    return launch_pdl("patchify_kernel", kern, blocks, threads, 0, stream, im, out, B, H, W);
+  }
+  const float* im = reinterpret_cast<const float*>(img);
+  const auto kern = patch == 8 ? patchify_kernel<8, float, MIRROR> : patchify_kernel<16, float, MIRROR>;
+  return launch_pdl("patchify_kernel", kern, blocks, threads, 0, stream, im, out, B, H, W);
 }
 
 extern "C" int stego_vit_patchify(const float* img, void* out_bf16, int B, int H, int W, int patch, void* stream_) {
@@ -236,9 +239,8 @@
                                   void* stream_) {
   cudaStream_t stream = reinterpret_cast<cudaStream_t>(stream_);
   STEGO_CHECK_ARG(x && cls_token && pos_embed && B > 0 && ntok > 0 && E > 0, "stego_vit_cls_rows: bad args");
-  cls_rows_kernel<<<(B * E + 255) / 256, 256, 0, stream>>>(x, cls_token, pos_embed, B, ntok, E);
-  STEGO_CHECK_LAUNCH("cls_rows_kernel");
-  return STEGO_OK;
+  return launch_pdl("cls_rows_kernel", cls_rows_kernel, (B * E + 255) / 256, 256, 0, stream, x, cls_token, pos_embed, B,
+                    ntok, E);
 }
 
 extern "C" int stego_layernorm_bf16(const float* x, const float* gamma, const float* beta, void* out_bf16, int rows,
@@ -249,17 +251,17 @@
   const int warps = 8;
   const int blocks = (rows + warps - 1) / warps;
   bf16* o = reinterpret_cast<bf16*>(out_bf16);
+  void (*kern)(const float*, const float*, const float*, bf16*, int, float, int);
   switch (E) {
-    case 384: layernorm_kernel<3><<<blocks, warps * 32, 0, stream>>>(x, gamma, beta, o, rows, eps, drop_cls_ntok); break;
-    case 768: layernorm_kernel<6><<<blocks, warps * 32, 0, stream>>>(x, gamma, beta, o, rows, eps, drop_cls_ntok); break;
-    case 128: layernorm_kernel<1><<<blocks, warps * 32, 0, stream>>>(x, gamma, beta, o, rows, eps, drop_cls_ntok); break;
+    case 384: kern = layernorm_kernel<3>; break;
+    case 768: kern = layernorm_kernel<6>; break;
+    case 128: kern = layernorm_kernel<1>; break;
     case 192:
     default:
       set_error("stego_layernorm_bf16: embed dim %d unsupported (128, 384, 768)", E);
       return STEGO_ERR_UNSUPPORTED;
   }
-  STEGO_CHECK_LAUNCH("layernorm_kernel");
-  return STEGO_OK;
+  return launch_pdl("layernorm_kernel", kern, blocks, warps * 32, 0, stream, x, gamma, beta, o, rows, eps, drop_cls_ntok);
 }
 
 extern "C" int stego_layernorm_gap(const float* x, const float* gamma, const float* beta, float* out, int B, int ntok,
diff --git a/stego_b200/dino/vision_transformer.py b/stego_b200/dino/vision_transformer.py
--- a/stego_b200/dino/vision_transformer.py
+++ b/stego_b200/dino/vision_transformer.py
@@ -205,7 +205,8 @@
         pos = self._pos_for(H, W, dev)
         rows = ops.patchify_tta(img, p) if mirror else ops.patchify(img, p)
         x = torch.empty(B * N, E, dtype=torch.float32, device=dev)
-        ops.gemm(rows, w["pe_w"], x, M=B * hw, N=E, K=3 * p * p, bias=w["pe_b"], residual=pos, row_div=hw)
+        ops.gemm(rows, w["pe_w"], x, M=B * hw, N=E, K=3 * p * p, bias=w["pe_b"], residual=pos, row_div=hw,
+                 frozen_b=True)
         ops.cls_rows(x, w["cls"], pos, B, N)
         y = torch.empty(B * N, E, dtype=torch.bfloat16, device=dev)
         qkv = torch.empty(B * N, 3 * E, dtype=torch.bfloat16, device=dev)
@@ -217,7 +218,7 @@
         for i, bw in enumerate(blocks[:-1] if stop_before_last else blocks):
             tap = taps is not None and depth - i <= taps.n
             ops.layernorm(x, bw["n1w"], bw["n1b"], y, eps=bw["eps1"])
-            ops.gemm(y, bw["qkv_w"], qkv, M=B * N, N=3 * E, K=E, bias=bw["qkv_b"])
+            ops.gemm(y, bw["qkv_w"], qkv, M=B * N, N=3 * E, K=E, bias=bw["qkv_b"], frozen_b=True)
             if tap:
                 taps.qkv.append(qkv.clone())
                 if taps.probs:
@@ -226,10 +227,10 @@
                 if taps.stop_at_last_probs and i == depth - 1:
                     break
             ops.attention(qkv, ao, B, N, E, heads)
-            ops.gemm(ao, bw["proj_w"], x, M=B * N, N=E, K=E, bias=bw["proj_b"], residual=x)
+            ops.gemm(ao, bw["proj_w"], x, M=B * N, N=E, K=E, bias=bw["proj_b"], residual=x, frozen_b=True)
             ops.layernorm(x, bw["n2w"], bw["n2b"], y, eps=bw["eps2"])
-            ops.gemm(y, bw["fc1_w"], hid, M=B * N, N=Hd, K=E, bias=bw["fc1_b"], act=ops.ACT_GELU)
-            ops.gemm(hid, bw["fc2_w"], x, M=B * N, N=E, K=Hd, bias=bw["fc2_b"], residual=x)
+            ops.gemm(y, bw["fc1_w"], hid, M=B * N, N=Hd, K=E, bias=bw["fc1_b"], act=ops.ACT_GELU, frozen_b=True)
+            ops.gemm(hid, bw["fc2_w"], x, M=B * N, N=E, K=Hd, bias=bw["fc2_b"], residual=x, frozen_b=True)
             if tap:
                 taps.x.append(x.clone())
         return x, (qkv if want_qkv else None)
@@ -299,7 +300,8 @@
         y = torch.empty(B * (N - 1), E, dtype=torch.bfloat16, device=x.device)
         ops.layernorm(x, bw["n1w"], bw["n1b"], y, eps=bw["eps1"], drop_cls_ntok=N)
         out = torch.empty(B * (N - 1), E, dtype=torch.bfloat16, device=x.device)
-        ops.gemm(y, bw["qkv_w"][E:2 * E], out, M=B * (N - 1), N=E, K=E, bias=bw["qkv_b"][E:2 * E])
+        ops.gemm(y, bw["qkv_w"][E:2 * E], out, M=B * (N - 1), N=E, K=E, bias=bw["qkv_b"][E:2 * E],
+                 frozen_b=True)
         return out.view(B, N - 1, E)
 
     @torch.no_grad()
diff --git a/stego_b200/ops.py b/stego_b200/ops.py
--- a/stego_b200/ops.py
+++ b/stego_b200/ops.py
@@ -12,7 +12,7 @@
 def gemm(a: torch.Tensor, b: torch.Tensor, out: torch.Tensor, *, M: int, N: int, K: int,
          a_mn: bool = False, b_mn: bool = False, bias: Optional[torch.Tensor] = None, act: int = ACT_NONE,
          residual: Optional[torch.Tensor] = None, row_div: int = 0, splits: int = 1,
-         atomic: bool = False) -> torch.Tensor:
+         atomic: bool = False, frozen_b: bool = False) -> torch.Tensor:
     _lib.require_cuda(a, b, out, bias, residual)
     assert a.dtype == torch.bfloat16 and b.dtype == torch.bfloat16
     assert a.dim() == 2 and b.dim() == 2 and out.dim() == 2
@@ -22,7 +22,8 @@
         assert bias.dtype == torch.float32 and bias.is_contiguous()
     if residual is not None:
         assert residual.dtype == torch.float32 and residual.stride(1) == 1
-    rc = _lib.load().stego_gemm_bf16(
+    lib = _lib.load()
+    rc = (lib.stego_gemm_bf16_frozen_b if frozen_b else lib.stego_gemm_bf16)(
         _lib.ptr(a), a.stride(0), int(a_mn), _lib.ptr(b), b.stride(0), int(b_mn), M, N, K,
         _lib.ptr(out), out.stride(0), int(out.dtype == torch.bfloat16), _lib.ptr(bias), act,
         _lib.ptr(residual), residual.stride(0) if residual is not None else 0, row_div, splits, int(atomic),
```
